# liamhebert/MultiModalDiscussionTransformer

Measured on AMD Instinct MI355X. Metric: discussion-tree comments/sec fwd+bwd, higher is better.
Workload: dtype bf16; 1 GPU; mDT-base (BERT-base + ViT-B/16 split 6+6, 6 executed graph layers, D768 H12 nb4 L100), 32 bushy 64-comment trees per GPU, 25% image comments, random-init weights, dropout 0.4/0.3/0.3 (run_train.sh:37), token lengths U{8..100} zero-padded to 100 (SURVEY.md §8d; mean 54.3 valid tokens), text side ragged: padded token positions are not computed (identical logits / gradients), last fusion layer comput; trees_per_gpu=32, parallelism=dp1, frozen_initial_encoders=False

## Files before the change

include/mdt_hip.h:

```cpp
#ifndef MDT_HIP_H
#define MDT_HIP_H

#include <stdint.h>

#ifdef __cplusplus
extern "C" {
#endif

#define MDT_ABI_VERSION 1

typedef enum { MDT_F32 = 0, MDT_BF16 = 1 } mdt_dtype;

typedef enum {
  MDT_OK = 0,
  MDT_ERR_ARG = -1,
  MDT_ERR_INVALID = MDT_ERR_ARG,
  MDT_ERR_UNSUPPORTED = -2,
  MDT_ERR_LAUNCH = -3
} mdt_status;

enum {
  MDT_EPI_BIAS = 1,
  MDT_EPI_GELU = 2,
  MDT_EPI_RESIDUAL = 4,
  MDT_EPI_DGELU = 8,
  MDT_EPI_ACCUM = 16,
  MDT_EPI_ATOMIC = 32,
  MDT_EPI_COLSUM = 128,
  MDT_EPI_AUX_GRAD = 256,
  MDT_EPI_MULAUX = 512,
  MDT_EPI_ASUM = 1024,
  MDT_EPI_DROPOUT = 64
};

int mdt_abi_version(void);
const char* mdt_last_error_string(void);
const char* mdt_last_route(void);
const char* mdt_source_hash(void);

int mdt_gemm(void* stream, int dtype, int out_dtype, int trans_a, int trans_b,
             int64_t M, int64_t N, int64_t K,
             const void* A, int64_t lda, const void* B, int64_t ldb,
             void* C, int64_t ldc, int epilogue, float alpha,
             const void* bias, const void* residual, int64_t ldr,
             void* aux, int64_t ldaux, int split_k, float drop_p, uint64_t drop_seed, float* colsum);
size_t mdt_gemm_tile_queue_bytes(void);
int mdt_gemm_set_tile_queue(void* zeroed_device_buffer, size_t bytes);
void mdt_reload_env(void);

int mdt_dropout(void* stream, int dtype, int64_t rows, int D, const void* x, int64_t ldx, void* y, int64_t ldy,
                float p, uint64_t seed);
int mdt_dropout_mask(void* stream, int64_t n, float p, uint64_t seed, uint8_t* mask);

enum { MDT_ACT_GELU = 0, MDT_ACT_RELU = 1, MDT_ACT_GELU_ACCURATE = 2, MDT_ACT_TANH = 3, MDT_ACT_LINEAR = 4 };
int mdt_act_fwd(void* stream, int dtype, int kind, int64_t rows, int N, const void* pre, int64_t ld_pre, void* h, int64_t ld_h,
                void* u, int64_t ld_u, float drop_p, uint64_t drop_seed);

int mdt_colsum(void* stream, int dtype, int64_t M, int64_t N, const void* X, int64_t ldx, float* out,
               const int32_t* row_weight);

int mdt_layernorm_fwd(void* stream, int dtype, int64_t rows, int D, const void* x, int64_t ldx,
                      const void* gamma, const void* beta, float eps,
                      void* y, int64_t ldy, float* mean, float* rstd);
int mdt_layernorm_fwd_q8(void* stream, int dtype, int64_t rows, int D, const void* x, int64_t ldx, const void* gamma,
                         const void* beta, float eps, void* y, int64_t ldy, float* mean, float* rstd, void* q8_out,
                         int64_t ld_q8, int q8_format, const float* q8_scale, float* q8_amax);
int mdt_layernorm_bwd(void* stream, int dtype, int64_t rows, int D, const void* dy, int64_t lddy,
                      const void* x, int64_t ldx, const void* gamma, const float* mean, const float* rstd,
                      const void* add, int64_t ldadd, void* dx, int64_t lddx, float* dgamma, float* dbeta,
                      void* dxd, int64_t lddxd, float drop_p, uint64_t drop_seed, float* colsum);

typedef struct {
  int dtype;
  int nseq, S, H, hd;
  int64_t seq_stride, pos_stride;
  float scale;
  const void* qkv; int64_t ld_qkv;
  void* out; int64_t ld_out;
  float* lse;
  const uint8_t* key_mask;
  const float* dense_bias;
  const float* attn_bias;
  const int32_t* spatial_pos;
  const void* sp_table;
  const void* virt;
  const uint8_t* key_pad;
  int num_spatial;
  float drop_p;
  uint64_t drop_seed;
  const int32_t* seq_offsets;
  int q_limit;
  const int32_t* seq_ids;
  int s_cap;
  int nseq_total;
} mdt_attn_fwd_args;
int mdt_attention_fwd(void* stream, const mdt_attn_fwd_args* a);

typedef struct {
  mdt_attn_fwd_args f;
  const void* dout; int64_t ld_dout;
  void* dqkv; int64_t ld_dqkv;
  float* d_dense_bias;
  float* d_sp_table;
  float* d_virt;
} mdt_attn_bwd_args;
int mdt_attention_bwd(void* stream, const mdt_attn_bwd_args* a);
int mdt_attention_route(const mdt_attn_bwd_args* a, int bwd, char* route, size_t route_bytes, int32_t geometry[2]);
int mdt_attention_mean_probs(void* stream, const mdt_attn_fwd_args* a, float* out);
int mdt_attention_head_weights(void* stream, const mdt_attn_fwd_args* a, int raw_scores, float* out);

int mdt_graph_attn_bias(void* stream, int dtype, int nseq, int S, int H, const float* attn_bias,
                        const int32_t* spatial_pos, const void* sp_table, const void* virt,
                        float* out);

int mdt_row_axpby(void* stream, int dtype, int64_t nrows, int D,
                  void* dst, int64_t ldd, const int32_t* di, int64_t d_inner, int64_t d_stride, int64_t d_off,
                  const void* a, int64_t lda, const int32_t* ai, int64_t a_inner, int64_t a_stride, int64_t a_off, float alpha,
                  const void* b, int64_t ldb, const int32_t* bi, int64_t b_inner, int64_t b_stride, int64_t b_off, float beta,
                  int accumulate);
int mdt_row_scatter_add_f32(void* stream, int dtype, int64_t nrows, int D, float* table, int64_t ldt,
                            const int32_t* idx, const void* src, int64_t lds, int64_t s_stride, int64_t s_off);

int mdt_bert_embed_sum(void* stream, int dtype, int64_t M, int L, const int32_t* ids, const int32_t* types,
                       const void* word, const void* pos, const void* type, int D,
                       void* out, int64_t ldo, int64_t out_seq_stride, int64_t out_off);

int mdt_bert_embed_rows(void* stream, int dtype, int64_t rows, const int32_t* ids, const int32_t* types,
                        const int32_t* pos_ids, const void* word, const void* pos, const void* type, int D,
                        void* out, int64_t ldo);
int mdt_bert_embed_ln_rows(void* stream, int dtype, int64_t rows, const int32_t* ids, const int32_t* types,
                           const int32_t* pos_ids, const void* word, const void* pos, const void* type, int D,
                           const void* gamma, const void* beta, float eps, void* xs, int64_t ldxs, void* y, int64_t ldy,
                           float* mean, float* rstd);

int mdt_vit_patchify(void* stream, int dtype, int I, int C, int HW, int p, const float* img, void* cols, int64_t ldc);
int mdt_vit_assemble(void* stream, int dtype, int I, int np, int D, const void* patches, int64_t ldp,
                     const void* cls, const void* pos, void* tokens, int64_t ldt, int64_t seq_stride, int64_t off);
int mdt_vit_patch_embed(void* stream, int I, int C, int HW, int p, const float* img, const void* w, int64_t ldw,
                        const void* bias, const void* cls, const void* pos, int D, void* tokens, int64_t ldt,
                        int64_t seq_stride, int64_t off);

int mdt_graph_node_feature(void* stream, int dtype, int B, int T, int D, const void* src, int64_t lds,
                           const int32_t* node_row, const int32_t* in_degree, const int32_t* out_degree,
                           const void* in_emb, const void* out_emb, const void* graph_token, void* x, int64_t ldx);

int mdt_tanh_fwd(void* stream, int dtype, int64_t n, const void* x, void* y);
int mdt_tanh_bwd(void* stream, int dtype, int64_t n, const void* y, const void* dy, void* dx);

int mdt_node_ce(void* stream, int dtype, int64_t M, int nlab, const void* logits, const int32_t* rows,
                const int32_t* targets, float w_neg, float w_pos, int fp16_loss, float grad_scale,
                float* out_loss, int32_t* counters, void* dlogits);

int mdt_gemm_fp8(void* stream, int a_format, int64_t M, int64_t N, int64_t K, const void* A, int64_t lda, const void* B,
                 int64_t ldb, void* C, int64_t ldc, int epilogue, const float* inv_scale_a, const float* inv_scale_b,
                 const void* bias, const void* residual, int64_t ldr, void* aux, int64_t ldaux, float drop_p,
                 uint64_t drop_seed, float* colsum);
int mdt_gemm_fp8_q8(void* stream, int a_format, int64_t M, int64_t N, int64_t K, const void* A, int64_t lda, const void* B,
                    int64_t ldb, void* C, int64_t ldc, int epilogue, const float* inv_scale_a, const float* inv_scale_b,
                    const void* bias, const void* residual, int64_t ldr, void* aux, int64_t ldaux, float drop_p,
                    uint64_t drop_seed, float* colsum, void* q8_out, int64_t ld_q8, int q8_format, const float* q8_scale,
                    float* q8_amax);
int mdt_fp8_quantize(void* stream, int src_dtype, int fmt, int64_t rows, int64_t cols, const void* src, int64_t ld_src,
                     void* dst, int64_t ld_dst, const float* scale_dev, float* amax_dev);
int mdt_fp8_scale_update(void* stream, int n, float* amax, float* scale, float* inv_scale, const float* fmt_max, float margin);

size_t mdt_contrastive_loss_workspace_bytes(int B, int D);
int mdt_contrastive_loss(void* stream, int dtype, int B, int D, const void* emb, int64_t ld, const float* y,
                         const float* hard_y, float scale, float soft_negative_weight, int adaptive, void* workspace,
                         float grad_scale, float* out_loss, int32_t* counters, void* d_emb, int64_t ldd);

int mdt_cast(void* stream, int src_dtype, int dst_dtype, int64_t n, const void* src, void* dst);
int mdt_transpose2d(void* stream, int src_dtype, int dst_dtype, int64_t rows, int64_t cols,
                    const void* src, int64_t lds, void* dst, int64_t ldd);

int mdt_adam_step(void* stream, int dtype, int64_t n, void* param, float* master, const float* grad, float* m,
                  float* v, float lr, float beta1, float beta2, float eps, float weight_decay, int step,
                  const float* grad_scale);

typedef struct {
  void* param;
  float* master;
  const float* grad;
  float* m;
  float* v;
  int64_t numel;
} mdt_adam_tensor;
int mdt_adam_step_multi(void* stream, int dtype, int n_tensors, const mdt_adam_tensor* table_dev,
                        const int64_t* chunk_first_dev, int64_t total_chunks, float lr, float beta1, float beta2,
                        float eps, float weight_decay, int step, const float* grad_scale);

typedef struct {
  float scale;
  float gnorm;
  float step_size;
  int32_t skip;
  int32_t applied;
  int32_t clipped;
  int32_t skipped;
  int32_t reserved;
} mdt_adam_guard;
int mdt_grad_sumsq_multi(void* stream, int n_tensors, const mdt_adam_tensor* table_dev, const int64_t* chunk_first_dev,
                         int64_t total_chunks, float* partials);
int mdt_grad_sumsq(void* stream, int64_t n, const float* grad, float* partials);
int mdt_grad_norm_finalize(void* stream, const float* partials, int64_t n_partials, float max_norm,
                           const float* grad_scale, float lr, float beta1, float beta2, int step, int reset,
                           mdt_adam_guard* guard);
int mdt_adam_step_guarded(void* stream, int dtype, int64_t n, void* param, float* master, const float* grad, float* m,
                          float* v, float lr, float beta1, float beta2, float eps, float weight_decay, int step,
                          const mdt_adam_guard* guard);
int mdt_adam_step_multi_guarded(void* stream, int dtype, int n_tensors, const mdt_adam_tensor* table_dev,
                                const int64_t* chunk_first_dev, int64_t total_chunks, float lr, float beta1, float beta2,
                                float eps, float weight_decay, int step, const mdt_adam_guard* guard);

int mdt_adam_step_ema(void* stream, int dtype, int64_t n, void* param, float* master, const float* grad, float* m,
                      float* v, float lr, float beta1, float beta2, float eps, float weight_decay, int step,
                      const float* grad_scale, float* ema, float ema_decay);
int mdt_adam_step_multi_ema(void* stream, int dtype, int n_tensors, const mdt_adam_tensor* table_dev,
                            const int64_t* chunk_first_dev, int64_t total_chunks, float lr, float beta1, float beta2,
                            float eps, float weight_decay, int step, const float* grad_scale, float* const* ema_dev,
                            float ema_decay);
int mdt_adam_step_ema_guarded(void* stream, int dtype, int64_t n, void* param, float* master, const float* grad, float* m,
                              float* v, float lr, float beta1, float beta2, float eps, float weight_decay, int step,
                              const mdt_adam_guard* guard, float* ema, float ema_decay);
int mdt_adam_step_multi_ema_guarded(void* stream, int dtype, int n_tensors, const mdt_adam_tensor* table_dev,
                                    const int64_t* chunk_first_dev, int64_t total_chunks, float lr, float beta1, float beta2,
                                    float eps, float weight_decay, int step, const mdt_adam_guard* guard, float* const* ema_dev,
                                    float ema_decay);
int mdt_ema_swap_multi(void* stream, int dtype, int n_tensors, const mdt_adam_tensor* table_dev, float* const* ema_dev,
                       const int64_t* chunk_first_dev, int64_t total_chunks, int restore);

typedef struct {
  float lr_scale;
  float weight_decay;
} mdt_adam_group;
int mdt_adam_step_multi_groups(void* stream, int dtype, int n_tensors, const mdt_adam_tensor* table_dev,
                               const int64_t* chunk_first_dev, int64_t total_chunks, float lr, float beta1, float beta2,
                               float eps, int step, const mdt_adam_group* groups_dev, const float* grad_scale,
                               const mdt_adam_guard* guard, float* const* ema_dev, float ema_decay);
int mdt_adam_step_group(void* stream, int dtype, int64_t n, void* param, float* master, const float* grad, float* m, float* v,
                        float lr, float beta1, float beta2, float eps, int step, float lr_scale, float weight_decay,
                        const float* grad_scale, const mdt_adam_guard* guard, float* ema, float ema_decay);

int mdt_sum_slices_f32(void* stream, int64_t rows, int64_t cols, int slices, const float* ws, int64_t ld_ws, int64_t slice_stride,
                       float* out, int64_t ldo, int accumulate);
size_t mdt_gemm_splitk_ordered_workspace_bytes(int64_t M, int64_t N, int split_k);
int mdt_gemm_splitk_ordered(void* stream, int dtype, int trans_a, int trans_b, int64_t M, int64_t N, int64_t K,
                            const void* A, int64_t lda, const void* B, int64_t ldb, float* C, int64_t ldc, float alpha,
                            int split_k, void* workspace, size_t workspace_bytes);
size_t mdt_colsum_ordered_workspace_bytes(int64_t M, int64_t N);
int mdt_colsum_ordered(void* stream, int dtype, int64_t M, int64_t N, const void* X, int64_t ldx, float* out,
                       const int32_t* row_weight, void* workspace, size_t workspace_bytes);
size_t mdt_layernorm_bwd_ordered_workspace_bytes(int64_t rows, int D);
int mdt_layernorm_bwd_ordered(void* stream, int dtype, int64_t rows, int D, const void* dy, int64_t lddy,
                              const void* x, int64_t ldx, const void* gamma, const float* mean, const float* rstd,
                              const void* add, int64_t ldadd, void* dx, int64_t lddx, float* dgamma, float* dbeta,
                              void* dxd, int64_t lddxd, float drop_p, uint64_t drop_seed, float* colsum,
                              void* workspace, size_t workspace_bytes);
int mdt_row_segment_sum_f32(void* stream, int dtype, int nseg, int D, float* table, int64_t ldt, const int32_t* seg_row,
                            const int32_t* seg_off, const int32_t* order, const void* src, int64_t lds, int64_t s_stride,
                            int64_t s_off);
// ... 40 lines not shown
```

multimodaldiscussiontransformer_amd/_lib.py:

```python
from __future__ import annotations

import ctypes as C
import os
import sys

import torch

_HERE = os.path.dirname(os.path.abspath(__file__))
LIB_PATH = os.path.join(_HERE, "libmdt_hip.so")

MDT_F32, MDT_BF16 = 0, 1
EPI_BIAS, EPI_GELU, EPI_RESIDUAL, EPI_DGELU, EPI_ACCUM, EPI_ATOMIC, EPI_DROPOUT, EPI_COLSUM = 1, 2, 4, 8, 16, 32, 64, 128
EPI_AUX_GRAD, EPI_MULAUX, EPI_ASUM = 256, 512, 1024
ACT_GELU, ACT_RELU, ACT_GELU_ACCURATE, ACT_TANH, ACT_LINEAR = 0, 1, 2, 3, 4

_vp, _i, _i64, _f = C.c_void_p, C.c_int, C.c_int64, C.c_float


class AttnFwdArgs(C.Structure):
    _fields_ = [
        ("dtype", _i), ("nseq", _i), ("S", _i), ("H", _i), ("hd", _i),
        ("seq_stride", _i64), ("pos_stride", _i64), ("scale", _f),
        ("qkv", _vp), ("ld_qkv", _i64), ("out", _vp), ("ld_out", _i64), ("lse", _vp),
        ("key_mask", _vp), ("dense_bias", _vp), ("attn_bias", _vp), ("spatial_pos", _vp),
        ("sp_table", _vp), ("virt", _vp), ("key_pad", _vp), ("num_spatial", _i),
        ("drop_p", _f), ("drop_seed", C.c_uint64), ("seq_offsets", _vp), ("q_limit", _i),
        ("seq_ids", _vp), ("s_cap", _i), ("nseq_total", _i),
    ]


class AttnBwdArgs(C.Structure):
    _fields_ = [
        ("f", AttnFwdArgs), ("dout", _vp), ("ld_dout", _i64), ("dqkv", _vp), ("ld_dqkv", _i64),
        ("d_dense_bias", _vp), ("d_sp_table", _vp), ("d_virt", _vp),
    ]


_SIGS = {
    "mdt_abi_version": ([], _i),
    "mdt_last_error_string": ([], C.c_char_p),
    "mdt_last_route": ([], C.c_char_p),
    "mdt_source_hash": ([], C.c_char_p),
    "mdt_gemm": ([_vp, _i, _i, _i, _i, _i64, _i64, _i64, _vp, _i64, _vp, _i64, _vp, _i64, _i, _f, _vp, _vp, _i64,
                  _vp, _i64, _i, _f, C.c_uint64, _vp], _i),
    "mdt_gemm_tile_queue_bytes": ([], C.c_size_t),
    "mdt_gemm_set_tile_queue": ([_vp, C.c_size_t], _i),
    "mdt_reload_env": ([], None),
    "mdt_dropout": ([_vp, _i, _i64, _i, _vp, _i64, _vp, _i64, _f, C.c_uint64], _i),
    "mdt_dropout_mask": ([_vp, _i64, _f, C.c_uint64, _vp], _i),
    "mdt_act_fwd": ([_vp, _i, _i, _i64, _i, _vp, _i64, _vp, _i64, _vp, _i64, _f, C.c_uint64], _i),
    "mdt_colsum": ([_vp, _i, _i64, _i64, _vp, _i64, _vp, _vp], _i),
    "mdt_layernorm_fwd": ([_vp, _i, _i64, _i, _vp, _i64, _vp, _vp, _f, _vp, _i64, _vp, _vp], _i),
    "mdt_layernorm_fwd_q8": ([_vp, _i, _i64, _i, _vp, _i64, _vp, _vp, _f, _vp, _i64, _vp, _vp, _vp, _i64, _i, _vp, _vp], _i),
    "mdt_layernorm_bwd": ([_vp, _i, _i64, _i, _vp, _i64, _vp, _i64, _vp, _vp, _vp, _vp, _i64, _vp, _i64, _vp, _vp,
                           _vp, _i64, _f, C.c_uint64, _vp], _i),
    "mdt_attention_fwd": ([_vp, C.POINTER(AttnFwdArgs)], _i),
    "mdt_attention_bwd": ([_vp, C.POINTER(AttnBwdArgs)], _i),
    "mdt_attention_route": ([C.POINTER(AttnBwdArgs), _i, C.c_char_p, C.c_size_t, C.POINTER(C.c_int32)], _i),
    "mdt_attention_mean_probs": ([_vp, C.POINTER(AttnFwdArgs), _vp], _i),
    "mdt_attention_head_weights": ([_vp, C.POINTER(AttnFwdArgs), _i, _vp], _i),
    "mdt_graph_attn_bias": ([_vp, _i, _i, _i, _i, _vp, _vp, _vp, _vp, _vp], _i),
    "mdt_row_axpby": ([_vp, _i, _i64, _i, _vp, _i64, _vp, _i64, _i64, _i64, _vp, _i64, _vp, _i64, _i64, _i64, _f,
                       _vp, _i64, _vp, _i64, _i64, _i64, _f, _i], _i),
    "mdt_row_scatter_add_f32": ([_vp, _i, _i64, _i, _vp, _i64, _vp, _vp, _i64, _i64, _i64], _i),
    "mdt_sum_slices_f32": ([_vp, _i64, _i64, _i, _vp, _i64, _i64, _vp, _i64, _i], _i),
    "mdt_gemm_splitk_ordered_workspace_bytes": ([_i64, _i64, _i], C.c_size_t),
    "mdt_gemm_splitk_ordered": ([_vp, _i, _i, _i, _i64, _i64, _i64, _vp, _i64, _vp, _i64, _vp, _i64, _f, _i, _vp, C.c_size_t], _i),
    "mdt_colsum_ordered_workspace_bytes": ([_i64, _i64], C.c_size_t),
    "mdt_colsum_ordered": ([_vp, _i, _i64, _i64, _vp, _i64, _vp, _vp, _vp, C.c_size_t], _i),
    "mdt_layernorm_bwd_ordered_workspace_bytes": ([_i64, _i], C.c_size_t),
    "mdt_layernorm_bwd_ordered": ([_vp, _i, _i64, _i, _vp, _i64, _vp, _i64, _vp, _vp, _vp, _vp, _i64, _vp, _i64, _vp, _vp,
                                   _vp, _i64, _f, C.c_uint64, _vp, _vp, C.c_size_t], _i),
    "mdt_row_segment_sum_f32": ([_vp, _i, _i, _i, _vp, _i64, _vp, _vp, _vp, _vp, _i64, _i64, _i64], _i),
    "mdt_attn_bias_grad_ordered_workspace_bytes": ([_i, _i, _i], C.c_size_t),
    "mdt_attn_bias_grad_ordered": ([_vp, _i, _i, _i, _i, _vp, _vp, _vp, _vp, _vp, C.c_size_t], _i),
    "mdt_float_atomic_launches": ([_i], _i64),
    "mdt_lora_down": ([_vp, _i, _i64, _i, _i, _vp, _i64, _vp, _i64, _vp, _i64, _f], _i),
    "mdt_lora_up_add": ([_vp, _i, _i64, _i, _i, _vp, _i64, _vp, _i64, _vp, _i64, _f], _i),
    "mdt_lora_up_add_drop": ([_vp, _i, _i64, _i, _i, _vp, _i64, _vp, _i64, _vp, _i64, _f, _f, C.c_uint64], _i),
    "mdt_lora_up_add_mul": ([_vp, _i, _i64, _i, _i, _vp, _i64, _vp, _i64, _vp, _i64, _vp, _i64, _f], _i),
    "mdt_lora_up_act": ([_vp, _i, _i, _i64, _i, _i, _vp, _i64, _vp, _i64, _vp, _i64, _vp, _i64, _vp, _i64, _f, _f, C.c_uint64], _i),
    "mdt_lora_wgrad_slab_rows": ([], _i),
    "mdt_lora_wgrad_workspace_bytes": ([_i64, _i, _i], C.c_size_t),
    "mdt_lora_wgrad": ([_vp, _i, _i64, _i, _i, _vp, _i64, _vp, _i64, _vp, _i64, _f, _vp, C.c_size_t], _i),
    "mdt_bert_embed_sum": ([_vp, _i, _i64, _i, _vp, _vp, _vp, _vp, _vp, _i, _vp, _i64, _i64, _i64], _i),
    "mdt_bert_embed_rows": ([_vp, _i, _i64, _vp, _vp, _vp, _vp, _vp, _vp, _i, _vp, _i64], _i),
    "mdt_bert_embed_ln_rows": ([_vp, _i, _i64, _vp, _vp, _vp, _vp, _vp, _vp, _i, _vp, _vp, _f, _vp, _i64, _vp, _i64, _vp, _vp], _i),
    "mdt_vit_patchify": ([_vp, _i, _i, _i, _i, _i, _vp, _vp, _i64], _i),
    "mdt_vit_assemble": ([_vp, _i, _i, _i, _i, _vp, _i64, _vp, _vp, _vp, _i64, _i64, _i64], _i),
    "mdt_vit_patch_embed": ([_vp, _i, _i, _i, _i, _vp, _vp, _i64, _vp, _vp, _vp, _i, _vp, _i64, _i64, _i64], _i),
    "mdt_graph_node_feature": ([_vp, _i, _i, _i, _i, _vp, _i64, _vp, _vp, _vp, _vp, _vp, _vp, _vp, _i64], _i),
    "mdt_tanh_fwd": ([_vp, _i, _i64, _vp, _vp], _i),
    "mdt_tanh_bwd": ([_vp, _i, _i64, _vp, _vp, _vp], _i),
    "mdt_node_ce": ([_vp, _i, _i64, _i, _vp, _vp, _vp, _f, _f, _i, _f, _vp, _vp, _vp], _i),
    "mdt_gemm_fp8": ([_vp, _i, _i64, _i64, _i64, _vp, _i64, _vp, _i64, _vp, _i64, _i, _vp, _vp, _vp, _vp, _i64, _vp, _i64, _f,
                      C.c_uint64, _vp], _i),
    "mdt_gemm_fp8_q8": ([_vp, _i, _i64, _i64, _i64, _vp, _i64, _vp, _i64, _vp, _i64, _i, _vp, _vp, _vp, _vp, _i64, _vp, _i64, _f,
                         C.c_uint64, _vp, _vp, _i64, _i, _vp, _vp], _i),
    "mdt_fp8_quantize": ([_vp, _i, _i, _i64, _i64, _vp, _i64, _vp, _i64, _vp, _vp], _i),
    "mdt_fp8_scale_update": ([_vp, _i, _vp, _vp, _vp, _vp, _f], _i),
    "mdt_contrastive_loss_workspace_bytes": ([_i, _i], C.c_size_t),
    "mdt_contrastive_loss": ([_vp, _i, _i, _i, _vp, _i64, _vp, _vp, _f, _f, _i, _vp, _f, _vp, _vp, _vp, _i64], _i),
    "mdt_adam_step_multi": ([_vp, _i, _i, _vp, _vp, _i64, _f, _f, _f, _f, _f, _i, _vp], _i),
    "mdt_cast": ([_vp, _i, _i, _i64, _vp, _vp], _i),
    "mdt_transpose2d": ([_vp, _i, _i, _i64, _i64, _vp, _i64, _vp, _i64], _i),
    "mdt_adam_step": ([_vp, _i, _i64, _vp, _vp, _vp, _vp, _vp, _f, _f, _f, _f, _f, _i, _vp], _i),
    "mdt_grad_sumsq_multi": ([_vp, _i, _vp, _vp, _i64, _vp], _i),
    "mdt_grad_sumsq": ([_vp, _i64, _vp, _vp], _i),
    "mdt_grad_norm_finalize": ([_vp, _vp, _i64, _f, _vp, _f, _f, _f, _i, _i, _vp], _i),
    "mdt_adam_step_guarded": ([_vp, _i, _i64, _vp, _vp, _vp, _vp, _vp, _f, _f, _f, _f, _f, _i, _vp], _i),
    "mdt_adam_step_multi_guarded": ([_vp, _i, _i, _vp, _vp, _i64, _f, _f, _f, _f, _f, _i, _vp], _i),
    "mdt_adam_step_ema": ([_vp, _i, _i64, _vp, _vp, _vp, _vp, _vp, _f, _f, _f, _f, _f, _i, _vp, _vp, _f], _i),
    "mdt_adam_step_multi_ema": ([_vp, _i, _i, _vp, _vp, _i64, _f, _f, _f, _f, _f, _i, _vp, _vp, _f], _i),
    "mdt_adam_step_ema_guarded": ([_vp, _i, _i64, _vp, _vp, _vp, _vp, _vp, _f, _f, _f, _f, _f, _i, _vp, _vp, _f], _i),
    "mdt_adam_step_multi_ema_guarded": ([_vp, _i, _i, _vp, _vp, _i64, _f, _f, _f, _f, _f, _i, _vp, _vp, _f], _i),
    "mdt_adam_step_multi_groups": ([_vp, _i, _i, _vp, _vp, _i64, _f, _f, _f, _f, _i, _vp, _vp, _vp, _vp, _f], _i),
    "mdt_adam_step_group": ([_vp, _i, _i64, _vp, _vp, _vp, _vp, _vp, _f, _f, _f, _f, _i, _f, _f, _vp, _vp, _vp, _f], _i),
    "mdt_ema_swap_multi": ([_vp, _i, _i, _vp, _vp, _vp, _i64, _i], _i),
    "mdt_resize_plan_ksize": ([_i, _i], _i),
    "mdt_resize_plan": ([_i, _i, _vp, _vp, _i], _i),
    "mdt_image_norm_lut": ([C.c_double, _vp, _vp, _vp], _i),
    "mdt_image_preprocess": ([_vp, _i, _i, _vp, _vp, _vp, _vp, _vp, _i, _vp, _vp, _i], _i),
    "mdt_pack_structure": ([_i, _vp, _vp, _i, _i, _vp, _vp, _vp], _i),
    "mdt_pack_structure_ud": ([_i, _vp, _vp, _vp, _i, _i, _vp, _vp, _vp], _i),
}

EXPORTS = tuple(_SIGS)


class MdtError(RuntimeError):
    status = 0


class MdtUnsupported(MdtError):
    status = -2


def _load():
    if not os.path.exists(LIB_PATH):
        raise ImportError(
            f"{LIB_PATH} is missing: the HIP extension is the product path and has no fallback. "
            "Build it with `python -m multimodaldiscussiontransformer_amd.build` (hipcc, gfx950).")
    lib = C.CDLL(LIB_PATH)
    for name, (args, res) in _SIGS.items():
        fn = getattr(lib, name)
        fn.argtypes = args
        fn.restype = res
    if lib.mdt_abi_version() != 1:
        raise ImportError("libmdt_hip.so ABI version mismatch")
    skip = os.environ.get("MDT_SKIP_SOURCE_HASH") == "1"
    if skip and ("pytest" in sys.modules or os.environ.get("MDT_BENCH_OFFICIAL") == "1"):
        raise ImportError("MDT_SKIP_SOURCE_HASH=1 is refused under pytest and bench.py (bench.py --foreign-library for an A/B arm)")
    from .build import source_hash, hash_inputs_present
    if not skip and hash_inputs_present():
        built, here = lib.mdt_source_hash().decode(), source_hash()
        if built != here:
            raise ImportError(f"{LIB_PATH} was built from other sources (library {built[:16]}, csrc/ {here[:16]}): rebuild with "
                              "`python -m multimodaldiscussiontransformer_amd.build` (MDT_SKIP_SOURCE_HASH=1 overrides, for A/B runs of two builds)")
    return lib


lib = _load()


def reload_env():
    lib.mdt_reload_env()


def last_route() -> str:
    return lib.mdt_last_route().decode()


_TILE_QUEUE = None


def enable_dynamic_tile_queue(device="cuda"):
    global _TILE_QUEUE
    if _TILE_QUEUE is None:
        _TILE_QUEUE = torch.zeros(lib.mdt_gemm_tile_queue_bytes() // 4, dtype=torch.int32, device=device)
        check(lib.mdt_gemm_set_tile_queue(_TILE_QUEUE.data_ptr(), _TILE_QUEUE.numel() * 4), "mdt_gemm_set_tile_queue")
    return _TILE_QUEUE


def check(status: int, what: str = ""):
    if status != 0:
        e = (MdtUnsupported if status == -2 else MdtError)(f"{what}: status {status}: {lib.mdt_last_error_string().decode()}")
        e.status = status
        raise e


def dt(t: torch.Tensor) -> int:
    if t.dtype == torch.float32:
        return MDT_F32
    if t.dtype == torch.bfloat16:
        return MDT_BF16
    raise MdtError(f"unsupported dtype {t.dtype} (fp32 and bf16 only)")


def ptr(t) -> int:
    if t is None:
        return None
    if not t.is_cuda:
        raise MdtError("libmdt_hip operates on device tensors only (no CPU path)")
    return t.data_ptr()


def stream() -> int:
    if not torch.cuda.is_available():
        raise MdtError("no GPU visible: libmdt_hip is the only compute path (there is no CPU fallback)")
    return torch.cuda.current_stream().cuda_stream
```

multimodaldiscussiontransformer_amd/build.py:

```python
from __future__ import annotations

import os
import subprocess
import sys
from concurrent.futures import ThreadPoolExecutor

HERE = os.path.dirname(os.path.abspath(__file__))
CSRC = os.path.join(HERE, "csrc")
OUT = os.path.join(HERE, "libmdt_hip.so")
SOURCES = ["gemm.hip", "gemm_wgrad.hip", "gemm_f8.hip", "layernorm.hip", "attention.hip", "attention_v2.hip", "attention_long.hip", "rowops.hip", "elementwise.hip", "ordered.hip", "lora.hip", "activation.hip", "patch_embed.hip", "contrastive.hip", "fp8.hip", "optim.hip", "image.hip", "host.cpp"]
FLAGS = ["--offload-arch=gfx950", "-O3", "-fPIC", "-std=c++17", "-Wno-unused-result", "-ffp-contract=off"]
EXTRA = {"attention.hip": ["-mllvm", "-amdgpu-mfma-vgpr-form=1"], "attention_v2.hip": ["-mllvm", "-amdgpu-mfma-vgpr-form=1"],
         "gemm_wgrad.hip": ["-mllvm", "-amdgpu-mfma-vgpr-form=1"]}


def source_hash() -> str:
    import hashlib
    h = hashlib.sha256()
    files = sorted(os.path.join(CSRC, f) for f in os.listdir(CSRC) if f.endswith((".hip", ".cpp", ".hpp", ".h")))
    files.append(os.path.join(HERE, "..", "include", "mdt_hip.h"))
    for f in files:
        h.update(os.path.basename(f).encode() + b"\0")
        h.update(open(f, "rb").read())
    return h.hexdigest()


def hash_inputs_present() -> bool:
    return os.path.isdir(CSRC) and os.path.exists(os.path.join(HERE, "..", "include", "mdt_hip.h"))


def _stale(target, deps):
    if not os.path.exists(target):
        return True
    t = os.path.getmtime(target)
    return any(os.path.getmtime(d) > t for d in deps)


def build(verbose: bool = False, force: bool = False) -> str:
    hipcc = os.environ.get("HIPCC", "/opt/rocm/bin/hipcc")
    objdir = os.path.join(HERE, "build")
    os.makedirs(objdir, exist_ok=True)
    headers = [os.path.join(CSRC, "common.hpp"), os.path.join(CSRC, "attention_common.hpp"), os.path.join(CSRC, "gemm_tiles.hpp"), os.path.join(CSRC, "gemm_epilogue.hpp"),
               os.path.join(HERE, "..", "include", "mdt_hip.h")]
    objs, jobs = [], []
    for s in SOURCES:
        src = os.path.join(CSRC, s)
        obj = os.path.join(objdir, s.rsplit(".", 1)[0] + ".o")
        objs.append(obj)
        if force or _stale(obj, [src] + headers):
            lang = ["-x", "hip"] if s.endswith(".cpp") else []
            jobs.append([hipcc] + FLAGS + EXTRA.get(s, []) + lang + ["-c", src, "-o", obj])

    def run(cmd):
        if verbose:
            print(" ".join(cmd), flush=True)
        r = subprocess.run(cmd, capture_output=True, text=True)
        if r.returncode != 0:
            raise RuntimeError("hipcc failed:\n" + " ".join(cmd) + "\n" + r.stdout + r.stderr)
        return r

    with ThreadPoolExecutor(max_workers=4) as ex:
        list(ex.map(run, jobs))
    digest = source_hash()
    stamp_src = os.path.join(objdir, "source_hash.cpp")
    stamp_obj = os.path.join(objdir, "source_hash.o")
    text = f'extern "C" const char* mdt_source_hash(void) {{ return "{digest}"; }}\n'
    if not os.path.exists(stamp_src) or open(stamp_src).read() != text or not os.path.exists(stamp_obj):
        open(stamp_src, "w").write(text)
        run([hipcc, "-x", "c++", "-O1", "-fPIC", "-c", stamp_src, "-o", stamp_obj])
        jobs.append(None)
    if force or jobs or _stale(OUT, objs + [stamp_obj]):
        run([hipcc, "--offload-arch=gfx950", "-shared", "-fPIC", "-o", OUT] + objs + [stamp_obj])
    return OUT


if __name__ == "__main__":
    print(build(verbose=True, force="--force" in sys.argv))
```

multimodaldiscussiontransformer_amd/csrc/attention.hip:

```cpp
#include <type_traits>

#include <stdlib.h>

#include "attention_common.hpp"

namespace mdt {

template <typename T> struct MM;
template <> struct MM<float> {
  static constexpr int KS = 4;
  typedef float frag;
  static __device__ __forceinline__ f32x4 mma(frag a, frag b, f32x4 c) { return mfma_f32(a, b, c); }
};
template <> struct MM<bf16_t> {
  static constexpr int KS = 32;
  typedef bf16x8 frag;
  static __device__ __forceinline__ f32x4 mma(frag a, frag b, f32x4 c) { return mfma_bf16(a, b, c); }
};

template <typename T> struct Src {
  const T* p;
  int64_t ld;
  int rows;
};
// ... 471 lines not shown
  AttnPlan pl{};
  pl.bwd = bwd;
  pl.st_bias = a.attn_bias != nullptr;
  pl.drop = a.drop_p > 0.f;
  pl.binned = a.seq_ids != nullptr || a.s_cap > 0;
  pl.dense_only = (a.dense_bias != nullptr || p.d_dense_bias != nullptr) && !pl.st_bias;
  pl.cap = a.s_cap > 0 ? a.s_cap : a.S;
  pl.n_t = (pl.cap + 15) / 16;
  pl.nhist = (bwd && pl.st_bias) ? attn_hist_size(a.num_spatial) : 0;
  const bool bf = a.dtype == MDT_BF16;
  if (pl.binned) {
    if (a.S > 272 || !bf || a.hd != 64 || !a.seq_offsets) {
      set_error("attention: seq_ids / s_cap are for ragged bf16 launches with head_dim 64 and S <= 272");
      return refuse(pl);
    }
  } else if (a.S > 272) return plan_long(pl, a);
  if (!attn_head_dim_ok(a.hd)) {
    set_error(bf ? "attention(bf16): head_dim %d unsupported (16, 64, 96 or 128)" : "attention: head_dim %d unsupported (16, 64, 96 or 128)", a.hd);
    return refuse(pl);
  }
  if (bf && pl.dense_only && !attn_v1_fits(a.hd, a.S)) return plan_long(pl, a);
  const bool one_pass = a.hd == 64 && !pl.st_bias && !pl.dense_only && attn_one_pass_lds_bytes(pl.n_t) <= ATTN_LDS_MAX && pl.n_t <= 16;
  pl.rows_img = attn_one_pass_rows(pl.n_t);
  pl.ldq = attn_one_pass_ldq(pl.n_t);
  auto ok = [&](AttnRoute r) {
    switch (r) {
      case AttnRoute::v1: return !pl.binned && a.q_limit == 0 && attn_v1_fits(a.hd, a.S);
      case AttnRoute::v2: return !pl.binned && !pl.dense_only && a.q_limit == 0 && a.S <= 112;
      case AttnRoute::v3: return !pl.dense_only;
      case AttnRoute::v4: return one_pass;
      case AttnRoute::v4x: return one_pass && pl.n_t <= 2 * V4_EXACT_PAIRS;
      case AttnRoute::v5: return one_pass && pl.n_t > 8 && pl.rows_img * 8 <= 4 * 512;
      default: return false;
    }
  };
  if (!bf) pl.route = AttnRoute::v1;
  else if (!bwd) pl.route = pl.dense_only ? AttnRoute::v1 : AttnRoute::v2;
  else {
    const AttnRoute family = ok(AttnRoute::v5) ? AttnRoute::v5 : ok(AttnRoute::v4x) ? AttnRoute::v4x : one_pass ? AttnRoute::v4 : AttnRoute::v3;
    if (pl.binned) pl.route = family;
    else if (pl.dense_only) pl.route = AttnRoute::v1;
    else if (a.S > 256) pl.route = family;
    else if (a.S <= 80 && a.q_limit == 0 && pl.st_bias) pl.route = AttnRoute::v1;
    else if (!pl.drop && ok(AttnRoute::v2)) pl.route = AttnRoute::v2;
    else pl.route = family;
    const AttnRoute forced = switches().attn_bwd;
    if (forced != AttnRoute::none && ok(forced)) pl.route = forced;
  }
  switch (pl.route) {
    case AttnRoute::v1: {
      pl.rung = attn_rung<2, 5, 7, 9, 13, 17>((a.S + 15) / 16);
      if (!pl.rung) { set_error("attention: S=%d exceeds the 272-token limit of the single-pass kernel", a.S); return refuse(pl); }
      const size_t lds = attn_v1_lds_bytes(bf, a.hd, pl.rung, bwd, pl.nhist);
      if (lds > ATTN_LDS_MAX) {
        set_error(bwd ? "attention_bwd (v1): S=%d with head_dim %d needs %zu bytes of LDS" : "attention (v1): S=%d with head_dim %d needs %zu bytes of LDS", a.S, a.hd, lds);
        return refuse(pl);
      }
      if (!bf && bwd && a.hd > 64 && pl.rung == 17 && pl.st_bias && pl.drop) return plan_long(pl, a);
      break;
    }
    case AttnRoute::v2:
      pl.rung = attn_rung<2, 4, 5, 7, 9, 13, 17>(pl.n_t);
      if (!pl.rung) { set_error("attention_v2: S=%d exceeds 272", a.S); return refuse(pl); }
      if (bwd && pl.rung > 7) { set_error("attention_v2: backward supports S <= 112 (got %d)", a.S); return refuse(pl); }
      if (!bwd) pl.waves = attn_v2_fwd_waves(pl.rung, pl.st_bias);
      break;
    case AttnRoute::v3: {
      pl.tight = attn_v3_tight(a.hd, pl.cap);
      pl.s_pad = attn_v3_s_pad(pl.cap, pl.tight);
      const size_t lds = attn_v3_lds_bytes(a.hd, pl.s_pad, pl.tight, pl.nhist);
      if (lds > ATTN_LDS_MAX) { set_error("attention_bwd_v3: S=%d needs %zu bytes of LDS", pl.cap, lds); return refuse(pl); }
      pl.threads = (a.hd <= 64 && !pl.st_bias && pl.s_pad > 128) ? 512 : 256;
      break;
    }
    case AttnRoute::v5:
      pl.items = (int)((int64_t)a.H * a.nseq);
      pl.wgs = pl.items < device_cus() ? pl.items : device_cus();
      break;
    case AttnRoute::v4:
    case AttnRoute::v4x:
      pl.waves = pl.n_t <= 4 ? 4 : pl.n_t <= 8 ? 8 : 16;
      break;
    default: break;
  }
  return pl;
}

int attention_v1_launch(hipStream_t st, const AttnParams& p, const AttnPlan& pl) {
  return with_dtype(p.f.dtype, [&](auto t) { return with_head_dim(p.f.hd, [&](auto hd) { return with_flags(pl, [&](auto s, auto d) {
    return with_rung<2, 5, 7, 9, 13, 17>(pl.rung, [&](auto nt) {
      using T = typename decltype(t)::type;
      constexpr int HD = decltype(hd)::value, NT = decltype(nt)::value;
      constexpr bool STRUCT = decltype(s)::value, DROP = decltype(d)::value, BF = !std::is_same<T, float>::value;
      const size_t lds = attn_v1_lds_bytes(BF, HD, NT, pl.bwd, pl.nhist);
      const dim3 grid(p.f.H, p.f.nseq);
      if (!pl.bwd) return launch_route<attn_fwd_kernel<T, HD, NT, STRUCT, DROP>>("v1", grid, 256, lds, st, p);
      if constexpr (!BF && HD > 64 && NT == 17 && STRUCT && DROP) return attn_unplanned("the fp32 v1 backward of wide heads at 17 tiles with structural bias and dropout");
      else return launch_route<attn_bwd_kernel<T, HD, NT, STRUCT, DROP>>("v1", grid, 256, lds, st, p);
    });
  }); }); });
}

static bool attn_rows_aligned(int dtype, const void* base, int64_t ld) {
  return dtype == MDT_BF16 ? (ld % 8 == 0 && ((uintptr_t)base & 15) == 0) : ((uintptr_t)base & 3) == 0;
}

static int check_args(const mdt_attn_fwd_args& a) {
  MDT_CHECK_ARG(a.dtype == MDT_F32 || a.dtype == MDT_BF16, "attention: bad dtype %d", a.dtype);
  MDT_CHECK_ARG(a.nseq >= 0 && a.S > 0 && a.H > 0 && a.hd > 0, "attention: bad shape nseq=%d S=%d H=%d hd=%d", a.nseq,
                a.S, a.H, a.hd);
  MDT_CHECK_ARG(a.qkv && a.out && a.lse, "attention: null qkv / out / lse");
  MDT_CHECK_ARG(a.ld_qkv >= 3 * a.H * a.hd && a.ld_out >= a.H * a.hd, "attention: row strides too small");
  if (a.dtype == MDT_BF16) {
    MDT_CHECK_ARG(attn_rows_aligned(a.dtype, a.qkv, a.ld_qkv), "attention(bf16): qkv must be 16-byte aligned rows");
    MDT_CHECK_ARG(attn_rows_aligned(a.dtype, a.out, a.ld_out), "attention(bf16): out must be 16-byte aligned rows");
  } else {
    MDT_CHECK_ARG(attn_rows_aligned(a.dtype, a.qkv, a.ld_qkv), "attention(fp32): qkv must be 4-byte aligned");
    MDT_CHECK_ARG(attn_rows_aligned(a.dtype, a.out, a.ld_out), "attention(fp32): out must be 4-byte aligned");
  }
  if (a.attn_bias) MDT_CHECK_ARG(a.spatial_pos && a.sp_table && a.virt && a.num_spatial > 0, "attention: incomplete structural bias");
  MDT_CHECK_ARG(a.drop_p >= 0.f && a.drop_p < 1.f, "attention: dropout p=%f out of [0,1)", a.drop_p);
  if (a.seq_offsets)
    MDT_CHECK_ARG(a.pos_stride == 1 && !a.key_mask && !a.key_pad && !a.dense_bias && !a.attn_bias,
                  "attention: ragged sequences (seq_offsets) take no masks / biases and need pos_stride == 1");
  MDT_CHECK_ARG(a.s_cap >= 0 && a.s_cap <= a.S, "attention: s_cap=%d outside [0, S=%d]", a.s_cap, a.S);
  MDT_CHECK_ARG(!a.seq_ids || (a.seq_offsets && (a.nseq_total == 0 || a.nseq_total >= a.nseq)),
                "attention: seq_ids need seq_offsets (and nseq_total >= nseq)");
  MDT_CHECK_ARG(a.drop_p == 0.f || (uint64_t)(a.nseq_total > a.nseq ? a.nseq_total : a.nseq) * a.H * a.S * (a.S + 1) < (1ull << 32),
                "attention: dropout counters are 32-bit (nseq*H*S*(S+1) must stay below 2^32)");
  return MDT_OK;
}

static int checked_params(const mdt_attn_fwd_args& f, const mdt_attn_bwd_args* b, AttnParams& p) {
  if (int e = check_args(f)) return e;
  memset(&p, 0, sizeof(p));
  p.f = f;
  p.drop = make_drop(f.drop_p, f.drop_seed);
  if (!b) return MDT_OK;
  MDT_CHECK_ARG(b->dout && b->dqkv, "attention_bwd: null dout / dqkv");
  MDT_CHECK_ARG(b->ld_dqkv >= 3 * f.H * f.hd, "attention_bwd: ld_dqkv too small");
  MDT_CHECK_ARG(b->ld_dout >= f.H * f.hd, "attention_bwd: ld_dout too small");
  if (f.dtype == MDT_BF16) {
    MDT_CHECK_ARG(attn_rows_aligned(f.dtype, b->dout, b->ld_dout), "attention_bwd(bf16): dout must be 16-byte aligned rows");
    MDT_CHECK_ARG(attn_rows_aligned(f.dtype, b->dqkv, b->ld_dqkv), "attention_bwd(bf16): dqkv must be 16-byte aligned rows");
  } else {
    MDT_CHECK_ARG(attn_rows_aligned(f.dtype, b->dout, b->ld_dout), "attention_bwd(fp32): dout must be 4-byte aligned");
    MDT_CHECK_ARG(attn_rows_aligned(f.dtype, b->dqkv, b->ld_dqkv), "attention_bwd(fp32): dqkv must be 4-byte aligned");
  }
  p.dout = b->dout; p.ld_dout = b->ld_dout; p.dqkv = b->dqkv; p.ld_dqkv = b->ld_dqkv;
  p.d_dense_bias = b->d_dense_bias; p.d_sp_table = b->d_sp_table; p.d_virt = b->d_virt;
  return MDT_OK;
}

static int dispatch(hipStream_t st, const mdt_attn_fwd_args& f, const mdt_attn_bwd_args* b) {
  AttnParams p;
  if (int e = checked_params(f, b, p)) return e;
  if (p.d_sp_table || p.d_virt) note_float_atomic_launch();
  const AttnPlan pl = attn_plan(p, b != nullptr);
  if (pl.status != MDT_OK) return pl.status;
  switch (pl.route) {
    case AttnRoute::v1: return attention_v1_launch(st, p, pl);
    case AttnRoute::long_: return attention_long_launch(st, p, pl);
    default: return attention_v2_launch(st, p, pl);
  }
}

}

using namespace mdt;

extern "C" int mdt_attention_fwd(void* stream, const mdt_attn_fwd_args* a) {
  MDT_CHECK_ARG(a, "attention_fwd: null args");
  if (a->nseq == 0) return MDT_OK;
  return dispatch((hipStream_t)stream, *a, nullptr);
}

extern "C" int mdt_attention_bwd(void* stream, const mdt_attn_bwd_args* a) {
  MDT_CHECK_ARG(a, "attention_bwd: null args");
  if (a->f.nseq == 0) return MDT_OK;
  return dispatch((hipStream_t)stream, a->f, a);
}

extern "C" int mdt_attention_route(const mdt_attn_bwd_args* a, int bwd, char* route, size_t route_bytes, int32_t geometry[2]) {
  MDT_CHECK_ARG(a && route && route_bytes > 0 && geometry, "attention_route: null args");
  route[0] = 0;
  geometry[0] = geometry[1] = 0;
  AttnParams p;
  if (int e = checked_params(a->f, bwd ? a : nullptr, p)) return e;
  const AttnPlan pl = attn_plan(p, bwd != 0);
  if (pl.status != MDT_OK) return pl.status;
  snprintf(route, route_bytes, "%s", route_name(pl.route));
  switch (pl.route) {
    case AttnRoute::v1:
    case AttnRoute::v2: geometry[0] = pl.rung; geometry[1] = pl.waves; break;
    case AttnRoute::v3: geometry[0] = pl.s_pad; geometry[1] = pl.threads; break;
    case AttnRoute::v4:
    case AttnRoute::v4x: geometry[0] = pl.waves; break;
    default: break;
  }
  return MDT_OK;
}

extern "C" int mdt_attention_mean_probs(void* stream, const mdt_attn_fwd_args* a, float* out) {
  MDT_CHECK_ARG(a && out, "attention_mean_probs: null args");
  if (a->nseq == 0) return MDT_OK;
  if (int e = check_args(*a)) return e;
  MDT_CHECK_ARG(!a->seq_offsets, "attention_mean_probs: ragged sequences are not supported (module-level API only)");
  const int64_t n = (int64_t)a->nseq * a->S * a->S;
  const int grid = (int)((n + 255) / 256 > 8192 ? 8192 : (n + 255) / 256);
  return with_dtype(a->dtype, [&](auto t) {
    return launch_plain<attn_mean_probs_kernel<typename decltype(t)::type>>("attention_mean_probs", grid, 256, (hipStream_t)stream, *a, out);
  });
}

template <typename T, bool RAW>
__global__ __launch_bounds__(256) void attn_head_weights_kernel(mdt_attn_fwd_args a, float* out) {
  const int S = a.S, H = a.H, hd = a.hd;
  const int64_t n = (int64_t)a.nseq * H * S * S;
  for (int64_t i = (int64_t)blockIdx.x * 256 + threadIdx.x; i < n; i += (int64_t)gridDim.x * 256) {
    const int key = (int)(i % S), q = (int)((i / S) % S), h = (int)((i / ((int64_t)S * S)) % H), seq = (int)(i / ((int64_t)S * S * H));
    const T* qrow = (const T*)a.qkv + ((int64_t)seq * a.seq_stride + (int64_t)q * a.pos_stride) * a.ld_qkv + h * hd;
    const T* krow = (const T*)a.qkv + ((int64_t)seq * a.seq_stride + (int64_t)key * a.pos_stride) * a.ld_qkv + (int64_t)H * hd + h * hd;
    const BiasCtx bc = bias_ctx(a, seq, h, S);
    float v = key_only_bias<T>(bc, key);
    if (v == 0.f) {
      float dot = 0.f;
      for (int d = 0; d < hd; ++d) dot += to_f32(qrow[d]) * to_f32(krow[d]);
      v = dot * a.scale + (a.attn_bias ? pair_bias<T, true>(bc, q, key) : pair_bias<T, false>(bc, q, key));
    }
    if constexpr (RAW) {
      out[i] = v;
    } else {
      const float l = a.lse[((int64_t)seq * H + h) * S + q];
      out[i] = (v == -INFINITY || l == -INFINITY) ? 0.f : __expf(v - l);
    }
  }
}

extern "C" int mdt_attention_head_weights(void* stream, const mdt_attn_fwd_args* a, int raw_scores, float* out) {
  MDT_CHECK_ARG(a && out, "attention_head_weights: null args");
  if (a->nseq == 0) return MDT_OK;
  if (int e = check_args(*a)) return e;
  MDT_CHECK_ARG(!a->seq_offsets, "attention_head_weights: ragged sequences are not supported (module-level API only)");
  MDT_CHECK_ARG(raw_scores || a->lse, "attention_head_weights: probabilities need the forward's log-sum-exp");
  const int64_t n = (int64_t)a->nseq * a->H * a->S * a->S;
  const int grid = (int)((n + 255) / 256 > 8192 ? 8192 : (n + 255) / 256);
  hipStream_t st = (hipStream_t)stream;
  return with_dtype(a->dtype, [&](auto t) {
    using T = typename decltype(t)::type;
    return raw_scores ? launch_plain<attn_head_weights_kernel<T, true>>("attention_head_weights", grid, 256, st, *a, out)
                      : launch_plain<attn_head_weights_kernel<T, false>>("attention_head_weights", grid, 256, st, *a, out);
  });
}

extern "C" int mdt_graph_attn_bias(void* stream, int dtype, int nseq, int S, int H, const float* attn_bias,
                                   const int32_t* spatial_pos, const void* sp_table, const void* virt, float* out) {
  MDT_CHECK_ARG(attn_bias && spatial_pos && sp_table && virt && out, "graph_attn_bias: null pointer");
  if (nseq == 0) return MDT_OK;
  const int64_t n = (int64_t)nseq * H * S * S;
  const int grid = (int)((n + 255) / 256 > 8192 ? 8192 : (n + 255) / 256);
  hipStream_t st = (hipStream_t)stream;
  return with_dtype(dtype, [&](auto t) {
    using T = typename decltype(t)::type;
    return launch_plain<graph_attn_bias_kernel<T>>("graph_attn_bias", grid, 256, st, nseq, S, H, attn_bias, spatial_pos, (const T*)sp_table, (const T*)virt, out);
  });
}
```

multimodaldiscussiontransformer_amd/csrc/attention_common.hpp:

```cpp
#pragma once
#include "common.hpp"

namespace mdt {

struct AttnParams {
  mdt_attn_fwd_args f;
  DropCfg drop;
  const void* dout; int64_t ld_dout;
  void* dqkv; int64_t ld_dqkv;
  float* d_dense_bias; float* d_sp_table; float* d_virt;
};

struct BiasCtx {
  int seq, h, S, H;
  const uint8_t* key_mask;
  const uint8_t* key_pad;
  const float* dense;
  const float* attn_bias;
  const int32_t* sp;
  const void* table;
  const void* virt;
};
__device__ __forceinline__ BiasCtx bias_ctx(const mdt_attn_fwd_args& a, int seq, int h, int S) {
  return BiasCtx{seq, h, S, a.H, a.key_mask, a.key_pad, a.dense_bias, a.attn_bias, a.spatial_pos, a.sp_table, a.virt};
}

template <typename T>
struct AttnItem {
  int seq, S, SL, D;
  int64_t row0;
  const T* qkv; const T* dout; const T* out; T* dqkv;
  int64_t tld, dld, old_, gld;
};
template <typename T, int HD>
__device__ __forceinline__ AttnItem<T> attn_item(const AttnParams& P, int h, unsigned si) {
  const mdt_attn_fwd_args& a = P.f;
  const int seq = a.seq_ids ? a.seq_ids[si] : (int)si;
  const int SL = a.S, D = a.H * HD;
  const int S = a.seq_offsets ? a.seq_offsets[seq + 1] - a.seq_offsets[seq] : a.S;
  const int64_t row0 = a.seq_offsets ? (int64_t)a.seq_offsets[seq] : (int64_t)seq * a.seq_stride;
  const T* qkv = (const T*)a.qkv + row0 * a.ld_qkv + h * HD;
  const T* dout = (const T*)P.dout + row0 * P.ld_dout + h * HD;
  const T* out = (const T*)a.out + row0 * a.ld_out + h * HD;
  T* dqkv = (T*)P.dqkv + row0 * P.ld_dqkv + h * HD;
  return AttnItem<T>{seq, S, SL, D, row0, qkv, dout, out, dqkv, a.pos_stride * a.ld_qkv, a.pos_stride * P.ld_dout, a.pos_stride * a.ld_out,
                     a.pos_stride * P.ld_dqkv};
}

template <typename T>
__device__ __forceinline__ float key_only_bias(const BiasCtx& b, int key) {
  if (key >= b.S) return -INFINITY;
  if (b.key_mask && !b.key_mask[(int64_t)b.seq * b.S + key]) return -INFINITY;
  if (b.key_pad && b.key_pad[(int64_t)b.seq * b.S + key]) return -INFINITY;
  return 0.f;
}

template <typename T, bool STRUCT>
__device__ __forceinline__ float pair_bias(const BiasCtx& b, int q, int key) {
  float v = 0.f;
  if (b.dense) v += b.dense[(((int64_t)b.seq * b.H + b.h) * b.S + q) * b.S + key];
  if constexpr (STRUCT) {
    v += 2.0f * b.attn_bias[((int64_t)b.seq * b.S + q) * b.S + key];
    if (q >= 1 && key >= 1) {
      const int idx = b.sp[((int64_t)b.seq * (b.S - 1) + (q - 1)) * (b.S - 1) + (key - 1)];
      v += to_f32(((const T*)b.table)[(int64_t)idx * b.H + b.h]);
    } else {
      v += to_f32(((const T*)b.virt)[b.h]);
    }
  }
  return v;
}

constexpr float LOG2E = 1.4426950408889634f, LN2 = 0.6931471805599453f;

__device__ __forceinline__ uint32_t attn_row_pairs(int bh, int S, int q) {
  return (uint32_t)(bh * S + q) * (uint32_t)((S + 1) >> 1);
}
__device__ __forceinline__ uint32_t attn_drop_word(const DropCfg& d, uint32_t row_pairs, int key) {
  return drop_mix((row_pairs + (uint32_t)(key >> 1)) ^ d.key);
}
__device__ __forceinline__ bool drop_keep_lo(const DropCfg& d, uint32_t w) { return (w & 0xFFFFu) >= d.thresh; }
__device__ __forceinline__ bool drop_keep_hi(const DropCfg& d, uint32_t w) { return (w >> 16) >= d.thresh; }
__device__ __forceinline__ void attn_keep4_keys(const DropCfg& d, uint32_t pair, bool (&keep)[4]) {
  const uint32_t w0 = drop_mix(pair ^ d.key), w1 = drop_mix((pair + 1) ^ d.key);
  keep[0] = drop_keep_lo(d, w0); keep[1] = drop_keep_hi(d, w0);
  keep[2] = drop_keep_lo(d, w1); keep[3] = drop_keep_hi(d, w1);
}
__device__ __forceinline__ void attn_keep4_queries(const DropCfg& d, uint32_t kh, int qb, uint32_t s2h, int odd, bool (&keep)[4]) {
  const uint32_t ra = kh + (uint32_t)(qb + 2 * odd) * s2h;
  const uint32_t wa = drop_mix(ra ^ d.key), wb = drop_mix((ra + s2h) ^ d.key);
  const uint32_t pa = (uint32_t)__builtin_amdgcn_update_dpp(0, (int)wa, 0xB1, 0xF, 0xF, false);
  const uint32_t pb = (uint32_t)__builtin_amdgcn_update_dpp(0, (int)wb, 0xB1, 0xF, 0xF, false);
  const uint32_t w[4] = {odd ? pa : wa, odd ? pb : wb, odd ? wa : pa, odd ? wb : pb};
#pragma unroll
  for (int r = 0; r < 4; ++r) keep[r] = ((w[r] >> (16 * odd)) & 0xFFFFu) >= d.thresh;
}
__device__ __forceinline__ float attn_drop_scale(const DropCfg& d, int bh, int S, int q, int key) {
  const uint32_t w = attn_drop_word(d, attn_row_pairs(bh, S, q), key);
  return ((key & 1) ? drop_keep_hi(d, w) : drop_keep_lo(d, w)) ? d.inv_keep : 0.f;
}

__host__ __device__ inline int attn_hist_size(int num_spatial) { return (num_spatial + 1 + 3) & ~3; }
template <bool STRUCT>
__device__ __forceinline__ void attn_bias_grad_add(const AttnParams& P, float* s_hist, int seq, int h, int S, int q, int key, float ds) {
  const mdt_attn_fwd_args& a = P.f;
  if (P.d_dense_bias) P.d_dense_bias[(((int64_t)seq * a.H + h) * S + q) * S + key] = ds;
  if constexpr (STRUCT) {
    if (P.d_sp_table && ds != 0.f) {
      if (q >= 1 && key >= 1) {
        const int idx = a.spatial_pos[((int64_t)seq * (S - 1) + (q - 1)) * (S - 1) + (key - 1)];
        if (idx != 0) atomicAdd(s_hist + idx, ds);
      } else {
        atomicAdd(s_hist + a.num_spatial, ds);
      }
    }
  }
}
__device__ __forceinline__ void attn_bias_grad_flush(const AttnParams& P, const float* s_hist, int h, int tid, int nthr) {
  const mdt_attn_fwd_args& a = P.f;
  if (P.d_sp_table) {
    for (int i = tid; i <= a.num_spatial; i += nthr) {
      const float v = s_hist[i];
      if (v != 0.f) {
        if (i < a.num_spatial) atomicAdd(P.d_sp_table + (int64_t)i * a.H + h, v);
        else if (P.d_virt) atomicAdd(P.d_virt + h, v);
      }
    }
  }
}

constexpr int attn_v1_ld(int hd) { return hd >= 32 ? hd + 8 : hd; }
constexpr int attn_v2_ld(int hd, bool tight) { return hd < 32 ? hd : (hd <= 64 || tight) ? hd + 8 : hd + 16; }
template <int HD, bool TIGHT = false> constexpr int v2_ld = attn_v2_ld(HD, TIGHT);
template <int HD, int NT> constexpr int v2_ld_nt = v2_ld<HD, (HD == 128 && NT > 16)>;
constexpr int V4_EXACT_PAIRS = 3;
constexpr size_t ATTN_LDS_MAX = 160 * 1024;

constexpr bool attn_v1_fits(int hd, int S) { return hd < 128 || S <= 208; }

constexpr size_t attn_v1_lds_bytes(bool bf, int hd, int nt, bool bwd, int nhist) {
  const int s_pad32 = (nt * 16 + 31) & ~31, sld = s_pad32 + (bf ? 8 : 1);
  return (bwd ? (size_t)(2 * s_pad32 + nhist) * 4 : 0) + (size_t)4 * 16 * sld * (bf ? 2 : 4) + (bf ? (size_t)2 * s_pad32 * attn_v1_ld(hd) * 2 : 0);
}
constexpr size_t attn_v2_lds_bytes(int hd, int nt, bool bwd, int nhist) {
  const int s_pad = ((nt + 1) / 2) * 32;
  return (size_t)2 * s_pad * attn_v2_ld(hd, !bwd && hd == 128 && nt > 16) * 2 + (size_t)(bwd ? 3 : 1) * s_pad * 4 + (size_t)nhist * 4 + (bwd ? 0 : 16);
}
constexpr bool attn_v3_tight(int hd, int cap) { return hd == 128 && cap > 256; }
constexpr int attn_v3_s_pad(int cap, bool tight) { return tight ? (cap + 31) & ~31 : (cap + 63) & ~63; }
constexpr size_t attn_v3_lds_bytes(int hd, int s_pad, bool tight, int nhist) {
  return (size_t)2 * s_pad * attn_v2_ld(hd, tight) * 2 + (size_t)3 * s_pad * 4 + (size_t)nhist * 4;
}
constexpr int attn_one_pass_rows(int n_t) { return ((n_t + 1) / 2) * 32; }
constexpr int attn_one_pass_ldq(int n_t) { return (n_t & 1) ? 16 * n_t : 16 * n_t + 16; }
constexpr size_t attn_one_pass_lds_bytes(int n_t) {
  const size_t rows = attn_one_pass_rows(n_t), slabs = n_t <= 2 * V4_EXACT_PAIRS ? 7 : 0;
  return 2 * rows * attn_v2_ld(64, false) * 2 + (3 + slabs) * rows * 4 + (size_t)16 * n_t * attn_one_pass_ldq(n_t) * 2;
}
constexpr int attn_v2_fwd_waves(int nt, bool st_bias) { return (nt >= 13 && !st_bias) ? 8 : 4; }

struct AttnPlan {
  int status;
  AttnRoute route;
  bool bwd, st_bias, drop, binned, dense_only;
  int cap, n_t;
  int nhist;
  int rung;
  int s_pad, threads; bool tight;
  int rows_img, ldq, waves;
  int items, wgs;
};
AttnPlan attn_plan(const AttnParams& p, bool bwd);
int attention_v1_launch(hipStream_t st, const AttnParams& p, const AttnPlan& pl);
int attention_v2_launch(hipStream_t st, const AttnParams& p, const AttnPlan& pl);
int attention_long_launch(hipStream_t st, const AttnParams& p, const AttnPlan& pl);
inline int attn_unplanned(const char* what) { set_error("attention: %s is not instantiated and attn_plan never plans it", what); return MDT_ERR_UNSUPPORTED; }

constexpr bool attn_head_dim_ok(int hd) { return hd == 16 || hd == 64 || hd == 96 || hd == 128; }
template <typename F>
static int with_head_dim(int hd, F&& f) {
  switch (hd) {
    case 16: return f(std::integral_constant<int, 16>{});
    case 64: return f(std::integral_constant<int, 64>{});
    case 96: return f(std::integral_constant<int, 96>{});
    case 128: return f(std::integral_constant<int, 128>{});
  }
  return attn_unplanned("this head width");
}
template <typename F>
static int with_flags(const AttnPlan& pl, F&& f) {
  using T = std::true_type;
  using N = std::false_type;
  if (pl.st_bias && pl.drop) return f(T{}, T{});
  if (pl.st_bias) return f(T{}, N{});
  if (pl.drop) return f(N{}, T{});
  return f(N{}, N{});
}
template <int... RUNGS>
constexpr int attn_rung(int nt) {
  int r = 0;
  ((r = (r == 0 && nt <= RUNGS) ? RUNGS : r), ...);
  return r;
}
template <int... RUNGS, typename F>
static int with_rung(int rung, F&& f) {
  int e = MDT_ERR_UNSUPPORTED;
  const bool hit = ((rung == RUNGS ? (e = f(std::integral_constant<int, RUNGS>{}), true) : false) || ...);
  return hit ? e : attn_unplanned("this key-tile rung");
}

}
```

multimodaldiscussiontransformer_amd/csrc/attention_v2.hip:

```cpp
#include <type_traits>

#include "attention_common.hpp"

namespace mdt {

template <int HD> constexpr int v2_ks = (HD + 31) / 32;

template <int HD, int LD = v2_ld<HD>>
__device__ __forceinline__ void v2_stage(bf16_t* img, const bf16_t* g, int64_t g_ld, int S, int rows_pad, int tid, int nthr = 256) {
  constexpr int CH = HD / 8;
  for (int e = tid; e < rows_pad * CH; e += nthr) {
    const int r = e / CH, c = e - r * CH;
    bf16x8 v = bf16x8{0, 0, 0, 0, 0, 0, 0, 0};
    if (r < S) v = *(const bf16x8*)(g + r * g_ld + c * 8);
    *(bf16x8*)(img + r * LD + c * 8) = v;
  }
}

template <int HD, int NCH>
__device__ __forceinline__ void v2_stage_req(bf16x8 (&v)[NCH], const bf16_t* g, int64_t g_ld, int S, int tid, int nthr) {
  constexpr int CH = HD / 8;
#pragma unroll
  for (int j = 0; j < NCH; ++j) {
    const int e = tid + j * nthr, r = e / CH, c = e - r * CH;
    v[j] = *(const bf16x8*)(g + (r < S ? r : S - 1) * g_ld + c * 8);
  }
}
template <int HD, int NCH, int LD = v2_ld<HD>>
__device__ __forceinline__ void v2_stage_put(bf16_t* img, const bf16x8 (&v)[NCH], int S, int rows_pad, int tid, int nthr, bf16_t* spare) {
  constexpr int CH = HD / 8;
#pragma unroll
  for (int j = 0; j < NCH; ++j) {
    const int e = tid + j * nthr, r = e / CH, c = e - r * CH;
    bf16_t* dst = e < rows_pad * CH ? img + r * LD + c * 8 : spare;
    *(bf16x8*)dst = r < S ? v[j] : bf16x8{0, 0, 0, 0, 0, 0, 0, 0};
  }
}
struct KeyBytes { uint8_t km, kp; };
__device__ __forceinline__ KeyBytes key_only_bias_req(const BiasCtx& b, int key, const void* readable) {
  KeyBytes k{1, 0};
  if (b.key_mask || b.key_pad) {
    const int64_t at = (int64_t)b.seq * b.S + (key < b.S ? key : b.S - 1);
    const uint8_t* pm = b.key_mask ? b.key_mask + at : (const uint8_t*)readable;
    const uint8_t* pp = b.key_pad ? b.key_pad + at : (const uint8_t*)readable;
    const uint8_t m = *pm, q = *pp;
    k = KeyBytes{(uint8_t)(b.key_mask ? m : 1), (uint8_t)(b.key_pad ? q : 0)};
  }
  return k;
}
__device__ __forceinline__ float key_only_bias_of(const BiasCtx& b, int key, KeyBytes k) {
  return (key < b.S && k.km && !k.kp) ? 0.f : -INFINITY;
}

template <int HD>
__device__ __forceinline__ int v2_chunk(int lane) {
  static_assert(HD % 32 == 0 || HD == 16, "a head is whole K = 32 steps, or half of one");
  return HD % 32 == 0 ? lane >> 4 : (lane >> 4) & (HD / 8 - 1);
}
template <int HD, int LD = v2_ld<HD>>
__device__ __forceinline__ bf16x8 v2_frag_lds(const bf16_t* img, int rc0, int k0, int lane) {
  const bf16_t* a = img + (rc0 + (lane & 15)) * LD + k0 + 8 * v2_chunk<HD>(lane);
  return *(const __attribute__((address_space(3))) bf16x8*)LDS_PTR(a);
}
template <int HD>
__device__ __forceinline__ bf16x8 v2_frag_glb(const bf16_t* p, int64_t ld, int rows, int rc0, int k0, int lane) {
  int rc = rc0 + (lane & 15);
  if (rc > rows - 1) rc = rows - 1;
  bf16x8 v = *(const bf16x8*)(p + rc * ld + k0 + 8 * v2_chunk<HD>(lane));
  if constexpr (HD % 32 != 0) {
    if (k0 + 8 * (lane >> 4) >= HD) v = bf16x8{0, 0, 0, 0, 0, 0, 0, 0};
  }
  return v;
}
template <int HD, int LD = v2_ld<HD>>
__device__ __forceinline__ bf16x8 v2_frag_tr(const bf16_t* img, int t0, int d0, int lane) {
  const int g = lane >> 4, q4 = (lane >> 2) & 3, pp = lane & 3;
  const bf16_t* a = img + (t0 * 16 + 4 * g + q4) * LD + d0 + pp * 4;
  const bf16x4 lo = lds_read_tr16(a);
  const bf16x4 hi = lds_read_tr16(a + 16 * LD);
  return bf16x8{lo[0], lo[1], lo[2], lo[3], hi[0], hi[1], hi[2], hi[3]};
}
__device__ __forceinline__ bf16x8 v2_pack(const f32x4& lo, const f32x4& hi) {
  return bf16x8{(bf16_t)lo[0], (bf16_t)lo[1], (bf16_t)lo[2], (bf16_t)lo[3],
                (bf16_t)hi[0], (bf16_t)hi[1], (bf16_t)hi[2], (bf16_t)hi[3]};
}
__device__ __forceinline__ float col_max(float v) {
  v = fmaxf(v, __shfl_xor(v, 16, 64));
  return fmaxf(v, __shfl_xor(v, 32, 64));
}
__device__ __forceinline__ float col_sum(float v) {
  v += __shfl_xor(v, 16, 64);
  return v + __shfl_xor(v, 32, 64);
}

struct Row32 { bf16x8 a, b; };
__device__ __forceinline__ int rows4_off(int g) { return 16 * (g & 1) + 8 * (g >> 1); }
__device__ __forceinline__ Row32 rows4_exchange(const f32x4 (&x)[4], float scale) {
  uint32_t lo[4], hi[4];
#pragma unroll
  for (int d = 0; d < 4; ++d) {
    const bf16x4 v = bf16x4{(bf16_t)(x[d][0] * scale), (bf16_t)(x[d][1] * scale), (bf16_t)(x[d][2] * scale), (bf16_t)(x[d][3] * scale)};
    const uint2 u = __builtin_bit_cast(uint2, v);
    lo[d] = u.x;
    hi[d] = u.y;
  }
  asm volatile("s_nop 1\n\tv_permlane16_swap_b32 %0, %1" : "+v"(lo[0]), "+v"(lo[1]));
  asm volatile("s_nop 1\n\tv_permlane16_swap_b32 %0, %1" : "+v"(hi[0]), "+v"(hi[1]));
  asm volatile("s_nop 1\n\tv_permlane16_swap_b32 %0, %1" : "+v"(lo[2]), "+v"(lo[3]));
  asm volatile("s_nop 1\n\tv_permlane16_swap_b32 %0, %1" : "+v"(hi[2]), "+v"(hi[3]));
  Row32 r;
  r.a = __builtin_bit_cast(bf16x8, uint4{lo[0], hi[0], lo[1], hi[1]});
  r.b = __builtin_bit_cast(bf16x8, uint4{lo[2], hi[2], lo[3], hi[3]});
  return r;
}
__device__ __forceinline__ void rows4_store(bf16_t* row, const Row32& v, int g) {
  *(bf16x8*)(row + rows4_off(g)) = v.a;
  *(bf16x8*)(row + rows4_off(g) + 32) = v.b;
}
__device__ __forceinline__ void row_piece(bf16_t* p, const f32x4& x, float scale) {
  *(bf16x4*)p = bf16x4{(bf16_t)(x[0] * scale), (bf16_t)(x[1] * scale), (bf16_t)(x[2] * scale), (bf16_t)(x[3] * scale)};
}

template <bool STRUCT>
__device__ __forceinline__ void v2_p_ds(f32x4& sc, f32x4& dp, float scale2, float kb, const f32x4& l2v, const f32x4& dlv, const bool (&keep)[4],
                                        const BiasCtx* bc = nullptr, int qb = 0, int key = 0, bool kok = false) {
#pragma unroll
  for (int r = 0; r < 4; ++r) {
    float v = __builtin_fmaf(sc[r], scale2, kb);
    if constexpr (STRUCT) {
      const int q = qb + r;
      if (kok && q < bc->S) v = __builtin_fmaf(pair_bias<bf16_t, true>(*bc, q, key), LOG2E, v);
    }
    const float p = __builtin_amdgcn_exp2f(v - l2v[r]);
    const float dpv = keep[r] ? dp[r] : 0.f;
    sc[r] = keep[r] ? p : 0.f;
    dp[r] = p * (dpv - dlv[r]);
  }
}

template <int HD, int NT, bool STRUCT, bool DROP, int NW>
__global__ __launch_bounds__(NW * 64) void attn_fwd_v2_kernel(AttnParams P) {
  constexpr int ND = HD / 16, NP = (NT + 1) / 2, S_PAD = NP * 32, LD = v2_ld_nt<HD, NT>;
  extern __shared__ __attribute__((aligned(16))) char smem[];
  const mdt_attn_fwd_args& a = P.f;
  const int tid = threadIdx.x, lane = tid & 63, wave = tid >> 6;
  const int h = blockIdx.x, seq = a.seq_ids ? a.seq_ids[blockIdx.y] : (int)blockIdx.y;
  const int SL = a.S, D = a.H * HD;
  const int S = a.seq_offsets ? a.seq_offsets[seq + 1] - a.seq_offsets[seq] : a.S;
  const int64_t row0 = a.seq_offsets ? (int64_t)a.seq_offsets[seq] : (int64_t)seq * a.seq_stride;
  if (S > NT * 16 || S <= 0) return;
  const bf16_t* qkv = (const bf16_t*)a.qkv + row0 * a.ld_qkv + h * HD;
  const int64_t tld = a.pos_stride * a.ld_qkv;
  bf16_t* imgK = (bf16_t*)smem;
  bf16_t* imgV = imgK + S_PAD * LD;
  float* s_kb = (float*)(imgV + S_PAD * LD);
  BiasCtx bc{seq, h, S, a.H, a.key_mask, a.key_pad, a.dense_bias, a.attn_bias, a.spatial_pos, a.sp_table, a.virt};
  const int ntk = (S + 15) >> 4;
  constexpr int MAXT = (NT + NW - 1) / NW;
  int n_qt = (S + 15) >> 4;
  if (a.q_limit > 0 && ((a.q_limit + 15) >> 4) < n_qt) n_qt = (a.q_limit + 15) >> 4;
  constexpr bool PFQ = !(HD > 64 && STRUCT && NT >= 13);
  bf16x8 fq_all[PFQ ? MAXT : 1][v2_ks<HD>];
#pragma unroll
  for (int k = 0; k < (PFQ ? MAXT : 0); ++k) {
    const int qt_k = wave + NW * k;
    if (qt_k < n_qt) {
#pragma unroll
      for (int ks = 0; ks < v2_ks<HD>; ++ks) fq_all[k][ks] = v2_frag_glb<HD>(qkv, tld, S, qt_k * 16, ks * 32, lane);
    }
  }
  {
    constexpr int NCH = (S_PAD * (HD / 8) + NW * 64 - 1) / (NW * 64), NKB = (S_PAD + NW * 64 - 1) / (NW * 64);
    bf16x8 ck[NCH], cv[NCH];
    KeyBytes kbv[NKB];
    v2_stage_req<HD, NCH>(ck, qkv + D, tld, S, tid, NW * 64);
    v2_stage_req<HD, NCH>(cv, qkv + 2 * D, tld, S, tid, NW * 64);
#pragma unroll
    for (int j = 0; j < NKB; ++j) kbv[j] = key_only_bias_req(bc, tid + j * NW * 64, qkv);
    v2_stage_put<HD, NCH, LD>(imgK, ck, S, S_PAD, tid, NW * 64, (bf16_t*)(s_kb + S_PAD));
    v2_stage_put<HD, NCH, LD>(imgV, cv, S, S_PAD, tid, NW * 64, (bf16_t*)(s_kb + S_PAD));
#pragma unroll
    for (int j = 0; j < NKB; ++j)
      if (tid + j * NW * 64 < S_PAD) s_kb[tid + j * NW * 64] = key_only_bias_of(bc, tid + j * NW * 64, kbv[j]);
  }
  __syncthreads();
  const int drop_bh = seq * a.H + h;
  const float scale2 = a.scale * LOG2E;
  const int g = lane >> 4, c = lane & 15;
#pragma unroll
  for (int k = 0; k < MAXT; ++k) {
    const int qt = wave + NW * k;
    if (qt >= n_qt) break;
    const int q0 = qt * 16;
    const int q = q0 + c;
    const int qc = q < S ? q : S - 1;
    bf16x8 fq[v2_ks<HD>];
#pragma unroll
    for (int ks = 0; ks < v2_ks<HD>; ++ks) {
      if constexpr (PFQ) fq[ks] = fq_all[k][ks];
      else fq[ks] = v2_frag_glb<HD>(qkv, tld, S, q0, ks * 32, lane);
    }
    f32x4 sc[2 * NP];
#pragma unroll
    for (int t = 0; t < 2 * NP; ++t) sc[t] = f32x4{0.f, 0.f, 0.f, 0.f};
#pragma unroll
    for (int t = 0; t < NT; ++t) {
#pragma unroll
      for (int ks = 0; ks < v2_ks<HD>; ++ks) {
        sc[t] = mfma_bf16(v2_frag_lds<HD, LD>(imgK, t * 16, ks * 32, lane), fq[ks], sc[t]);
        if (ks == v2_ks<HD> - 1 && (t & 1)) __builtin_amdgcn_sched_barrier(0);
      }
    }
    float mx = -INFINITY;
#pragma unroll
    for (int t = 0; t < NT; ++t) {
      if (t >= ntk) continue;
      const f32x4 kb = *(const f32x4*)(s_kb + t * 16 + 4 * g);
#pragma unroll
      for (int r = 0; r < 4; ++r) {
        float v = __builtin_fmaf(sc[t][r], scale2, kb[r]);
        if constexpr (STRUCT) {
          const int key = t * 16 + 4 * g + r;
          if (key < S) v = __builtin_fmaf(pair_bias<bf16_t, true>(bc, qc, key), LOG2E, v);
        }
        sc[t][r] = v;
        mx = fmaxf(mx, v);
      }
    }
    mx = col_max(mx);
    const float mxc = (mx == -INFINITY) ? 0.f : mx;
    float sum = 0.f;
#pragma unroll
    for (int t = 0; t < NT; ++t) {
      if (t >= ntk) continue;
#pragma unroll
      for (int r = 0; r < 4; ++r) {
        const float e = __builtin_amdgcn_exp2f(sc[t][r] - mxc);
        sc[t][r] = e;
        sum += e;
      }
    }
    sum = col_sum(sum);
    if (g == 0 && q < S) a.lse[((int64_t)seq * a.H + h) * SL + q] = (sum > 0.f) ? (mxc + __builtin_amdgcn_logf(sum)) * LN2 : -INFINITY;
    float inv = (sum > 0.f) ? __builtin_amdgcn_rcpf(sum) : 0.f;
    if constexpr (DROP) {
      inv *= P.drop.inv_keep;
      const uint32_t rp = attn_row_pairs(drop_bh, SL, qc) + 2 * g;
#pragma unroll
      for (int t = 0; t < NT; ++t) {
        if (t >= ntk) continue;
        const uint32_t w0 = drop_mix((rp + 8 * t) ^ P.drop.key), w1 = drop_mix((rp + 8 * t + 1) ^ P.drop.key);
        sc[t][0] = drop_keep_lo(P.drop, w0) ? sc[t][0] : 0.f;
        sc[t][1] = drop_keep_hi(P.drop, w0) ? sc[t][1] : 0.f;
        sc[t][2] = drop_keep_lo(P.drop, w1) ? sc[t][2] : 0.f;
        sc[t][3] = drop_keep_hi(P.drop, w1) ? sc[t][3] : 0.f;
      }
    }
    f32x4 o[ND];
#pragma unroll
    for (int d = 0; d < ND; ++d) o[d] = f32x4{0.f, 0.f, 0.f, 0.f};
#pragma unroll
    for (int pi = 0; pi < NP; ++pi) {
      if (2 * pi >= ntk) continue;
      const bf16x8 fp = v2_pack(sc[2 * pi], sc[2 * pi + 1]);
#pragma unroll
      for (int d = 0; d < ND; ++d) o[d] = mfma_bf16(v2_frag_tr<HD, LD>(imgV, 2 * pi, d * 16, lane), fp, o[d]);
      __builtin_amdgcn_sched_barrier(0);
    }
    if constexpr (ND == 4) {
      const Row32 ov = rows4_exchange(o, inv);
      if (q < S) {
        bf16_t* orow = (bf16_t*)a.out + (row0 + (int64_t)q * a.pos_stride) * a.ld_out + h * HD + rows4_off(g);
        *(bf16x8*)orow = ov.a;
// ... 561 lines not shown
  const float scale2 = a.scale * LOG2E;
  const int n_tq = (a.q_limit > 0 && ((a.q_limit + 15) >> 4) < n_t) ? (a.q_limit + 15) >> 4 : n_t;
  const int n_pair_q = (n_tq + 1) >> 1, n_pair_k = (n_t + 1) >> 1;

  const int odd = c & 1;
  const uint32_t base_rp = (uint32_t)(drop_bh * SL) * s2h;
  if (kt < n_t) {
    const int key = key0 + c;
    const bool kok = key < S;
    const float kb = s_kb[key];
    const uint32_t kh = base_rp + (uint32_t)(key >> 1);
    bf16_t* ds_row = dsT + (key0 + c) * ldq + 4 * g;
    f32x4 dv[ND], dk[ND];
#pragma unroll
    for (int d = 0; d < ND; ++d) { dv[d] = f32x4{0.f, 0.f, 0.f, 0.f}; dk[d] = f32x4{0.f, 0.f, 0.f, 0.f}; }
    if constexpr (EXACT) {
      f32x4 pA[V4_EXACT_PAIRS][2], dA[V4_EXACT_PAIRS][2];
      unsigned keepA[V4_EXACT_PAIRS];
#pragma unroll
      for (int pr = 0; pr < V4_EXACT_PAIRS; ++pr) {
        keepA[pr] = 0xFFu;
#pragma unroll
        for (int t = 0; t < 2; ++t) { pA[pr][t] = f32x4{0.f, 0.f, 0.f, 0.f}; dA[pr][t] = f32x4{0.f, 0.f, 0.f, 0.f}; }
        if (pr < n_pair_q) {
          const int t0 = 2 * pr;
#pragma unroll
          for (int t = 0; t < 2; ++t)
#pragma unroll
            for (int ks = 0; ks < v2_ks<HD>; ++ks) {
              pA[pr][t] = mfma_bf16(v2_frag_lds<HD>(img0, (t0 + t) * 16, ks * 32, lane), fk[ks], pA[pr][t]);
              dA[pr][t] = mfma_bf16(v2_frag_lds<HD>(img1, (t0 + t) * 16, ks * 32, lane), fv[ks], dA[pr][t]);
            }
#pragma unroll
          for (int t = 0; t < 2; ++t) {
            const int qb = (t0 + t) * 16 + 4 * g;
            const f32x4 l2v = *(const f32x4*)(s_lse + qb);
            bool keep[4] = {true, true, true, true};
            if constexpr (DROP) {
              attn_keep4_queries(P.drop, kh, qb, s2h, odd, keep);
#pragma unroll
              for (int r = 0; r < 4; ++r)
                if (!keep[r]) keepA[pr] &= ~(1u << (4 * t + r));
            }
            float x[4];
#pragma unroll
            for (int r = 0; r < 4; ++r) {
              const float v = __builtin_fmaf(pA[pr][t][r], scale2, kb);
              const float p = __builtin_amdgcn_exp2f(v - l2v[r]);
              const float dpv = keep[r] ? dA[pr][t][r] : 0.f;
              pA[pr][t][r] = p;
              dA[pr][t][r] = dpv;
              x[r] = row16_sum_dpp(p * dpv);
            }
            if (c == 0) *(f32x4*)(s_delta + kt * rows_img + qb) = f32x4{x[0], x[1], x[2], x[3]};
          }
        }
      }
      __syncthreads();
#pragma unroll
      for (int pr = 0; pr < V4_EXACT_PAIRS; ++pr) {
        if (pr < n_pair_q) {
          const int t0 = 2 * pr;
          f32x4 sc[2], dp[2];
#pragma unroll
          for (int t = 0; t < 2; ++t) {
            f32x4 dlv = *(const f32x4*)(s_delta + (t0 + t) * 16 + 4 * g);
            for (int w = 1; w < n_t; ++w) dlv += *(const f32x4*)(s_delta + w * rows_img + (t0 + t) * 16 + 4 * g);
#pragma unroll
            for (int r = 0; r < 4; ++r) {
              const float p = pA[pr][t][r];
              dp[t][r] = p * (dA[pr][t][r] - dlv[r]);
              sc[t][r] = (keepA[pr] >> (4 * t + r)) & 1u ? p : 0.f;
            }
          }
          const bf16x8 fp = v2_pack(sc[0], sc[1]);
          const bf16x8 fs = v2_pack(dp[0], dp[1]);
          onepass_put_ds(ds_row + t0 * 16, fs, t0 + 1 < n_tq);
#pragma unroll
          for (int d = 0; d < ND; ++d) {
            dv[d] = mfma_bf16(v2_frag_tr<HD>(img1, t0, d * 16, lane), fp, dv[d]);
            dk[d] = mfma_bf16(v2_frag_tr<HD>(img0, t0, d * 16, lane), fs, dk[d]);
          }
        }
      }
    }
    for (int pr = 0; pr < (EXACT ? 0 : n_pair_q); ++pr) {
      const int t0 = 2 * pr;
      f32x4 sc[2], dp[2];
#pragma unroll
      for (int t = 0; t < 2; ++t) { sc[t] = f32x4{0.f, 0.f, 0.f, 0.f}; dp[t] = f32x4{0.f, 0.f, 0.f, 0.f}; }
#pragma unroll
      for (int t = 0; t < 2; ++t)
#pragma unroll
        for (int ks = 0; ks < v2_ks<HD>; ++ks) {
          sc[t] = mfma_bf16(v2_frag_lds<HD>(img0, (t0 + t) * 16, ks * 32, lane), fk[ks], sc[t]);
          dp[t] = mfma_bf16(v2_frag_lds<HD>(img1, (t0 + t) * 16, ks * 32, lane), fv[ks], dp[t]);
        }
      __builtin_amdgcn_sched_barrier(0);
#pragma unroll
      for (int t = 0; t < 2; ++t) {
        const int qb = (t0 + t) * 16 + 4 * g;
        const f32x4 l2v = *(const f32x4*)(s_lse + qb);
        const f32x4 dlv = *(const f32x4*)(s_delta + qb);
        bool keep[4] = {true, true, true, true};
        if constexpr (DROP) attn_keep4_queries(P.drop, kh, qb, s2h, odd, keep);
        v2_p_ds<false>(sc[t], dp[t], scale2, kb, l2v, dlv, keep);
      }
      const bf16x8 fp = v2_pack(sc[0], sc[1]);
      const bf16x8 fs = v2_pack(dp[0], dp[1]);
      onepass_put_ds(ds_row + t0 * 16, fs, t0 + 1 < n_tq);
#pragma unroll
      for (int d = 0; d < ND; ++d) {
        dv[d] = mfma_bf16(v2_frag_tr<HD>(img1, t0, d * 16, lane), fp, dv[d]);
        dk[d] = mfma_bf16(v2_frag_tr<HD>(img0, t0, d * 16, lane), fs, dk[d]);
      }
      __builtin_amdgcn_sched_barrier(0);
    }
    static_assert(ND == 4, "rows4_exchange: 64-column rows");
    const Row32 kv = rows4_exchange(dk, a.scale * ik), vv = rows4_exchange(dv, ik);
    if (kok) {
      rows4_store(dqkv + (int64_t)key * gld + D, kv, g);
      rows4_store(dqkv + (int64_t)key * gld + 2 * D, vv, g);
    }
  } else if constexpr (EXACT) {
    __syncthreads();
  }
  __syncthreads();
  if (kt < n_t) onepass_put_k<HD>(img0, fk, kt, lane);
  __syncthreads();
  for (int qt = wave; qt < n_tq; qt += nw) {
    const int q = qt * 16 + c;
    f32x4 dq[ND];
#pragma unroll
    for (int d = 0; d < ND; ++d) dq[d] = f32x4{0.f, 0.f, 0.f, 0.f};
    for (int pk = 0; pk < n_pair_k; ++pk) {
      const bf16x8 fs = v2_frag_tr_ld(dsT, ldq, 2 * pk, qt * 16, lane, 2 * pk + 1 < n_t);
#pragma unroll
      for (int d = 0; d < ND; ++d) dq[d] = mfma_bf16(v2_frag_tr<HD>(img0, 2 * pk, d * 16, lane), fs, dq[d]);
    }
    const Row32 qv = rows4_exchange(dq, a.scale * ik);
    if (q < S) rows4_store(dqkv + (int64_t)q * gld, qv, g);
  }
}

template <int HD, bool DROP>
__global__ __launch_bounds__(1024) __attribute__((amdgpu_waves_per_eu(4, 4))) void attn_bwd_v4_kernel(AttnParams P, int rows_img, int ldq) {
  attn_bwd_v4_body<HD, DROP, false>(P, rows_img, ldq);
}
template <int HD, bool DROP>
__global__ __launch_bounds__(512) void attn_bwd_v4x_kernel(AttnParams P, int rows_img, int ldq) {
  attn_bwd_v4_body<HD, DROP, true>(P, rows_img, ldq);
}

template <int HD, bool DROP, int NU>
__device__ __forceinline__ void v5_phase1(const AttnParams& P, const bf16_t* img0, const bf16_t* img1, const float* s_kb, const float* s_lse,
                                          const float* s_delta, bf16_t* dsT, int ldq, const bf16x8 (&wk)[2][v2_ks<HD>], const bf16x8 (&wv)[2][v2_ks<HD>],
                                          int wave, int lane, int S, int SL, int drop_bh, int n_tq, bf16_t* dqkv, int64_t gld, int D, float ik) {
  constexpr int ND = HD / 16;
  const mdt_attn_fwd_args& a = P.f;
  const int g = lane >> 4, c = lane & 15, odd = c & 1;
  const uint32_t s2h = (uint32_t)((SL + 1) >> 1);
  const float scale2 = a.scale * LOG2E;
  const uint32_t base_rp = (uint32_t)(drop_bh * SL) * s2h;
  const int n_pair_q = (n_tq + 1) >> 1;
  int key[NU];
  float kb[NU];
  uint32_t kh[NU];
  bf16_t* ds_row[NU];
  f32x4 dv[NU][ND], dk[NU][ND];
#pragma unroll
  for (int u = 0; u < NU; ++u) {
    key[u] = (wave + 8 * u) * 16 + c;
    kb[u] = s_kb[key[u]];
    kh[u] = base_rp + (uint32_t)(key[u] >> 1);
    ds_row[u] = dsT + key[u] * ldq + 4 * g;
#pragma unroll
    for (int d = 0; d < ND; ++d) { dv[u][d] = f32x4{0.f, 0.f, 0.f, 0.f}; dk[u][d] = f32x4{0.f, 0.f, 0.f, 0.f}; }
  }
  for (int pr = 0; pr < n_pair_q; ++pr) {
    const int t0 = 2 * pr;
    f32x4 sc[NU][2], dp[NU][2];
#pragma unroll
    for (int u = 0; u < NU; ++u)
#pragma unroll
      for (int t = 0; t < 2; ++t) { sc[u][t] = f32x4{0.f, 0.f, 0.f, 0.f}; dp[u][t] = f32x4{0.f, 0.f, 0.f, 0.f}; }
#pragma unroll
    for (int t = 0; t < 2; ++t)
#pragma unroll
      for (int ks = 0; ks < v2_ks<HD>; ++ks) {
        const bf16x8 aq = v2_frag_lds<HD>(img0, (t0 + t) * 16, ks * 32, lane), ao = v2_frag_lds<HD>(img1, (t0 + t) * 16, ks * 32, lane);
#pragma unroll
        for (int u = 0; u < NU; ++u) {
          sc[u][t] = mfma_bf16(aq, wk[u][ks], sc[u][t]);
          dp[u][t] = mfma_bf16(ao, wv[u][ks], dp[u][t]);
        }
      }
    bf16x8 fp[NU], fs[NU];
    {
      f32x4 l2v[2], dlv[2];
#pragma unroll
      for (int t = 0; t < 2; ++t) {
        const int qb = (t0 + t) * 16 + 4 * g;
        l2v[t] = *(const f32x4*)(s_lse + qb);
        dlv[t] = *(const f32x4*)(s_delta + qb);
      }
#pragma unroll
      for (int u = 0; u < NU; ++u) {
#pragma unroll
        for (int t = 0; t < 2; ++t) {
          const int qb = (t0 + t) * 16 + 4 * g;
          bool keep[4] = {true, true, true, true};
          if constexpr (DROP) attn_keep4_queries(P.drop, kh[u], qb, s2h, odd, keep);
          v2_p_ds<false>(sc[u][t], dp[u][t], scale2, kb[u], l2v[t], dlv[t], keep);
        }
        fp[u] = v2_pack(sc[u][0], sc[u][1]);
        fs[u] = v2_pack(dp[u][0], dp[u][1]);
        onepass_put_ds(ds_row[u] + t0 * 16, fs[u], t0 + 1 < n_tq);
      }
    }
#pragma unroll
    for (int d = 0; d < ND; ++d) {
      const bf16x8 to = v2_frag_tr<HD>(img1, t0, d * 16, lane), tq = v2_frag_tr<HD>(img0, t0, d * 16, lane);
#pragma unroll
      for (int u = 0; u < NU; ++u) {
        dv[u][d] = mfma_bf16(to, fp[u], dv[u][d]);
        dk[u][d] = mfma_bf16(tq, fs[u], dk[u][d]);
      }
    }
  }
  static_assert(ND == 4, "rows4_exchange: 64-column rows");
#pragma unroll
  for (int u = 0; u < NU; ++u) {
    const Row32 kv = rows4_exchange(dk[u], a.scale * ik), vv = rows4_exchange(dv[u], ik);
    if (key[u] < S) {
      rows4_store(dqkv + (int64_t)key[u] * gld + D, kv, g);
      rows4_store(dqkv + (int64_t)key[u] * gld + 2 * D, vv, g);
    }
  }
}

__device__ __forceinline__ int v5_opaque(int x) {
  asm volatile("" : "+v"(x));
  return x;
}
__device__ __forceinline__ int v5_sload(const int* p) {
  int v;
  asm volatile("s_load_dword %0, %1, 0x0\n\ts_waitcnt lgkmcnt(0)" : "=s"(v) : "s"(p));
  return v;
}

template <int HD, bool DROP>
__global__ __launch_bounds__(512) __attribute__((amdgpu_waves_per_eu(2, 2))) void attn_bwd_v5_kernel(AttnParams P, int rows_img, int ldq, int n_items) {
  constexpr int NCH = 4;
  extern __shared__ __attribute__((aligned(16))) char smem[];
  const mdt_attn_fwd_args& a = P.f;
  const int tid = threadIdx.x, lane = tid & 63, wave = __builtin_amdgcn_readfirstlane(tid >> 6);
  const int SL = a.S, D = a.H * HD;
  const int64_t tld = a.pos_stride * a.ld_qkv, dld = a.pos_stride * P.ld_dout, old_ = a.pos_stride * a.ld_out, gld = a.pos_stride * P.ld_dqkv;
  bf16_t* img0 = (bf16_t*)smem;
  bf16_t* img1 = img0 + rows_img * v2_ld<HD>;
  float* s_kb = (float*)(img1 + rows_img * v2_ld<HD>);
  float* s_lse = s_kb + rows_img;
  float* s_delta = s_lse + rows_img;
  bf16_t* dsT = (bf16_t*)(s_delta + rows_img);
  const float ik = DROP ? P.drop.inv_keep : 1.0f, rik = 1.0f / ik;

  int seq, h, S, n_t, rows_live, q_rows;
  int64_t row0;
  auto item_of = [&](int it_) {
    const int it = __builtin_amdgcn_readfirstlane(it_);
    const int si = it / a.H;
    h = it - si * a.H;
    seq = a.seq_ids ? v5_sload(a.seq_ids + si) : si;
    if (a.seq_offsets) {
      const int o0 = v5_sload(a.seq_offsets + seq), o1 = v5_sload(a.seq_offsets + seq + 1);
      S = o1 - o0;
      row0 = o0;
    } else {
      S = a.S;
      row0 = (int64_t)seq * a.seq_stride;
    }
    n_t = (S + 15) >> 4;
    rows_live = ((n_t + 1) >> 1) * 32;
    if (rows_live > rows_img || S <= 0) { S = 0; n_t = 0; rows_live = 0; }
    q_rows = (a.q_limit > 0 && ((a.q_limit + 15) & ~15) < S) ? ((a.q_limit + 15) & ~15) : S;
  };
  bf16x8 cq[NCH], cg[NCH], co[NCH];
  float lv = 0.f;
  KeyBytes kbv{1, 0};
  bf16x8 wk[2][v2_ks<HD>], wv[2][v2_ks<HD>];
  auto request_rows = [&](int tid) {
    if (S > 0) {
      const bf16_t* qkv = (const bf16_t*)a.qkv + row0 * a.ld_qkv + h * HD;
      const bf16_t* dout = (const bf16_t*)P.dout + row0 * P.ld_dout + h * HD;
      const bf16_t* outp = (const bf16_t*)a.out + row0 * a.ld_out + h * HD;
      onepass_request<HD, NCH, true>(cq, cg, co, lv, kbv, a, bias_ctx(a, seq, h, S), qkv, dout, outp, tld, dld, old_, SL, q_rows, rows_live, tid, 512);
    }
  };
  auto request_frags = [&](int tid) {
    if (S > 0) {
      const int lane = tid & 63, wave = tid >> 6;
      const bf16_t* qkv = (const bf16_t*)a.qkv + row0 * a.ld_qkv + h * HD;

#pragma unroll
      for (int u = 0; u < 2; ++u)
#pragma unroll
        for (int ks = 0; ks < v2_ks<HD>; ++ks) {
          wk[u][ks] = v2_frag_glb<HD>(qkv + D, tld, S, (wave + 8 * u) * 16, ks * 32, lane);
          wv[u][ks] = v2_frag_glb<HD>(qkv + 2 * D, tld, S, (wave + 8 * u) * 16, ks * 32, lane);
        }
    }
  };

  int it = blockIdx.x;
  if (it >= n_items) return;
  item_of(it);
  request_rows(tid);
  request_frags(tid);
  for (;;) {
    const int cS = S, c_nt = n_t, c_rows = rows_live, c_qrows = q_rows, c_seq = seq, c_h = h;
    const int64_t c_row0 = row0;
    const int tid1 = v5_opaque(tid);
    onepass_stage<HD, NCH>(img0, img1, s_kb, s_lse, s_delta, cq, cg, co, lv, kbv, bias_ctx(a, c_seq, c_h, cS), c_qrows, c_rows, rik, tid1, 512);
#pragma unroll
    for (int u = 0; u < 2; ++u)
#pragma unroll
      for (int ks = 0; ks < v2_ks<HD>; ++ks) asm volatile("" ::"v"(wk[u][ks]), "v"(wv[u][ks]));
    __syncthreads();
    const int nxt = it + (int)gridDim.x;
    const bool more = nxt < n_items;
    if (more) { item_of(nxt); request_rows(v5_opaque(tid)); }
    bf16_t* dqkv = (bf16_t*)P.dqkv + c_row0 * P.ld_dqkv + c_h * HD;
    const int n_tq = (a.q_limit > 0 && ((a.q_limit + 15) >> 4) < c_nt) ? (a.q_limit + 15) >> 4 : c_nt;
    const int lane1 = v5_opaque(lane);
    if (wave + 8 < c_nt) v5_phase1<HD, DROP, 2>(P, img0, img1, s_kb, s_lse, s_delta, dsT, ldq, wk, wv, wave, lane1, cS, SL, c_seq * a.H + c_h, n_tq, dqkv, gld, D, ik);
    else if (wave < c_nt) v5_phase1<HD, DROP, 1>(P, img0, img1, s_kb, s_lse, s_delta, dsT, ldq, wk, wv, wave, lane1, cS, SL, c_seq * a.H + c_h, n_tq, dqkv, gld, D, ik);
    __syncthreads();
    const int tid2 = v5_opaque(tid), lane2 = tid2 & 63;
#pragma unroll
    for (int u = 0; u < 2; ++u)
      if (wave + 8 * u < c_nt) onepass_put_k<HD>(img0, wk[u], wave + 8 * u, lane2);
    if (more) request_frags(tid2);
    __syncthreads();
    onepass_phase2<HD>(img0, dsT, ldq, dqkv, gld, cS, c_nt, n_tq, wave, 8, v5_opaque(lane), a.scale * ik);
    if (!more) break;
    it = nxt;
    __syncthreads();
  }
}

template <bool DROP>
static int launch_one_pass(hipStream_t st, const AttnParams& p, const AttnPlan& pl) {
  const dim3 grid(p.f.H, p.f.nseq);
  const size_t lds = attn_one_pass_lds_bytes(pl.n_t);
  if (pl.route == AttnRoute::v5) return launch_route<attn_bwd_v5_kernel<64, DROP>>("v5", dim3((unsigned)pl.wgs), 512, lds, st, p, pl.rows_img, pl.ldq, pl.items);
  if (pl.route == AttnRoute::v4x) return launch_route<attn_bwd_v4x_kernel<64, DROP>>("v4x", grid, pl.waves * 64, lds, st, p, pl.rows_img, pl.ldq);
  return launch_route<attn_bwd_v4_kernel<64, DROP>>("v4", grid, pl.waves * 64, lds, st, p, pl.rows_img, pl.ldq);
}

template <int HD, bool STRUCT, bool DROP>
static int launch_v3(hipStream_t st, const AttnParams& p, const AttnPlan& pl) {
  if constexpr (HD == 64 && !STRUCT) {
    if (pl.route != AttnRoute::v3) return launch_one_pass<DROP>(st, p, pl);
  }
  const size_t lds = attn_v3_lds_bytes(HD, pl.s_pad, pl.tight, pl.nhist);
  const dim3 grid(p.f.H, p.f.nseq);
  if constexpr (HD > 64) {
    if (pl.tight) return launch_route<attn_bwd_v3_tight_kernel<HD, STRUCT, DROP>>("v3", grid, pl.threads, lds, st, p, pl.s_pad);
    return launch_route<attn_bwd_v3_kernel<HD, STRUCT, DROP>>("v3", grid, pl.threads, lds, st, p, pl.s_pad);
  } else if constexpr (STRUCT) return launch_route<attn_bwd_v3_kernel<HD, true, DROP>>("v3", grid, pl.threads, lds, st, p, pl.s_pad);
  else return launch_route<attn_bwd_v3_occ4_kernel<HD, DROP>>("v3", grid, pl.threads, lds, st, p, pl.s_pad);
}

template <int HD, int NT, bool STRUCT, bool DROP, bool BWD>
static int launch_v2(hipStream_t st, const AttnParams& p, const AttnPlan& pl) {
  const size_t lds = attn_v2_lds_bytes(HD, NT, BWD, pl.nhist);
  const dim3 grid(p.f.H, p.f.nseq);
  if constexpr (BWD && NT > 7) return attn_unplanned("the v2 backward past 112 keys");
  else if constexpr (BWD) return launch_route<attn_bwd_v2_kernel<HD, NT, STRUCT, DROP>>("v2", grid, 256, lds, st, p);
  else {
    constexpr int NWF = attn_v2_fwd_waves(NT, STRUCT);
    return launch_route<attn_fwd_v2_kernel<HD, NT, STRUCT, DROP, NWF>>("v2", grid, NWF * 64, lds, st, p);
  }
}

int attention_v2_launch(hipStream_t st, const AttnParams& p, const AttnPlan& pl) {
  return with_head_dim(p.f.hd, [&](auto hd) { return with_flags(pl, [&](auto s, auto d) {
    constexpr int HD = decltype(hd)::value;
    constexpr bool STRUCT = decltype(s)::value, DROP = decltype(d)::value;
    if (pl.route != AttnRoute::v2) return launch_v3<HD, STRUCT, DROP>(st, p, pl);
    return with_rung<2, 4, 5, 7, 9, 13, 17>(pl.rung, [&](auto nt) {
      constexpr int NT = decltype(nt)::value;
      return pl.bwd ? launch_v2<HD, NT, STRUCT, DROP, true>(st, p, pl) : launch_v2<HD, NT, STRUCT, DROP, false>(st, p, pl);
    });
  }); });
}

}
```

multimodaldiscussiontransformer_amd/engine.py:

```python
from __future__ import annotations

import os

import contextlib
import threading
import weakref
from dataclasses import dataclass
from typing import Callable, List, Optional, Sequence

import torch

from . import fp8 as F8
from . import ops


_DETERMINISTIC = os.environ.get("MDT_DETERMINISTIC", "0") == "1"


def set_deterministic(on: bool) -> None:
    global _DETERMINISTIC
    if on and F8.ACTIVE is not None:
        raise NotImplementedError("deterministic mode with fp8 GEMMs: the fp8 path has no ordered reductions (disable fp8 first)")
    _DETERMINISTIC = bool(on)

# ... 152 lines not shown
        finally:
            self._leave_side()
            self.record(self._enter_side)

    def _crossing(self, v: "Var", t: torch.Tensor):
        if self.side is not None and v.side != _SS.side_active:
            t.record_stream(self.side if v.side else self._main)

    def next_seed(self) -> int:
        if self._seed_base is None:
            self._seed_base = int(torch.randint(0, 2 ** 62, (1,)).item())
        self._seed_ctr += 1
        return (self._seed_base + 0x9E3779B97F4A7C15 * self._seed_ctr) & 0x7FFFFFFFFFFFFFFF

    def record(self, bwd: Callable[[], None]):
        if not self.inference:
            self.ops.append(bwd)

    def adjoint(self, o: "Var", bwd: Callable[[torch.Tensor], None], take: bool = True):
        def run():
            g = o.grad
            if take:
                o.grad = None
            if g is not None:
                bwd(g)

        self.record(run)

    def pgrad(self, p: torch.nn.Parameter) -> Optional[torch.Tensor]:
        if p is None or not p.requires_grad:
            return None
        if self.use_main_grad:
            g = getattr(p, "main_grad", None)
            if g is None:
                raise RuntimeError("use_main_grad=True but a trainable parameter has no .main_grad buffer")
            return g
        g = self.tmp_grads.get(id(p))
        if g is None:
            g = torch.zeros(p.shape, dtype=torch.float32, device=p.device)
            self.tmp_grads[id(p)] = g
        return g

    def grad_buf(self, v: Var) -> torch.Tensor:
        if v.grad is None:
            if self.side is not None and v.side and not _SS.side_active:
                with torch.cuda.stream(self.side):
                    v.grad = torch.zeros_like(v.data)
                torch.cuda.current_stream().wait_stream(self.side)
            else:
                v.grad = torch.zeros_like(v.data)
                self._crossing(v, v.grad)
        return v.grad

    def add_grad(self, v: Var, g: torch.Tensor):
        if not v.needs_grad:
            return
        if v.grad is None:
            v.grad = g
            self._crossing(v, g)
        else:
            ops.row_axpby(v.grad, v.grad.shape[0], a=g, accumulate=True)

    def backward(self):
        try:
            while self.ops:
                self.ops.pop()()
        finally:
            self._leave_side()
        self.ops = []
        self.sync_streams()
        if F8.ACTIVE is not None:
            F8.ACTIVE.end_of_step()

    def sync_streams(self):
        if self.side is not None:
            torch.cuda.current_stream().wait_stream(self.side)


@dataclass
class LoraSlot:
    A: torch.nn.Parameter
    Bt: torch.nn.Parameter
    scale: float = 1.0


@dataclass
class BlockParams:
    qkv_w: torch.nn.Parameter
    qkv_b: torch.nn.Parameter
    o_w: torch.nn.Parameter
    o_b: torch.nn.Parameter
    ln1_w: torch.nn.Parameter
    ln1_b: torch.nn.Parameter
    fc1_w: torch.nn.Parameter
    fc1_b: torch.nn.Parameter
    fc2_w: torch.nn.Parameter
    fc2_b: torch.nn.Parameter
    ln2_w: torch.nn.Parameter
    ln2_b: torch.nn.Parameter
    lora_A: Optional[torch.nn.Parameter] = None
    lora_Bt: Optional[torch.nn.Parameter] = None
    lora_cols: Optional[tuple] = None
    lora_scale: float = 1.0
    lora_o: Optional[LoraSlot] = None
    lora_fc1: Optional[LoraSlot] = None
    lora_fc2: Optional[LoraSlot] = None

    def dense_lora(self):
        return [s for s in (self.lora_o, self.lora_fc1, self.lora_fc2) if s is not None]

    def all(self):
        base = [self.qkv_w, self.qkv_b, self.o_w, self.o_b, self.ln1_w, self.ln1_b, self.fc1_w, self.fc1_b,
                self.fc2_w, self.fc2_b, self.ln2_w, self.ln2_b]
        if self.lora_A is not None:
            base = base + [self.lora_A, self.lora_Bt]
        return base + [p for s in self.dense_lora() for p in (s.A, s.Bt)]


@dataclass
class AttnSpec:
    nseq: int
    S: int
    H: int
    seq_stride: Optional[int] = None
    pos_stride: int = 1
    scale: Optional[float] = None
    key_mask: Optional[torch.Tensor] = None
    dense_bias: Optional[torch.Tensor] = None
    dense_bias_var: Optional[Var] = None
    attn_bias: Optional[torch.Tensor] = None
    spatial_pos: Optional[torch.Tensor] = None
    sp_table: Optional[torch.nn.Parameter] = None
    virt: Optional[torch.nn.Parameter] = None
    key_pad: Optional[torch.Tensor] = None
    seq_offsets: Optional[torch.Tensor] = None
    q_limit: int = 0
    bins: Optional[list] = None

    def kwargs(self):
        return dict(seq_stride=self.seq_stride, pos_stride=self.pos_stride, scale=self.scale, key_mask=self.key_mask,
                    seq_offsets=self.seq_offsets, q_limit=self.q_limit, bins=self.bins,
                    dense_bias=self.dense_bias, attn_bias=self.attn_bias, spatial_pos=self.spatial_pos,
                    sp_table=None if self.sp_table is None else self.sp_table.data,
                    virt=None if self.virt is None else self.virt.data.view(-1), key_pad=self.key_pad)


def _split_k(n_out: int, k_out: int, red: int) -> int:
    tiles = ((n_out + 127) // 128) * ((k_out + 127) // 128)
    s = max(1, 1024 // max(1, tiles))
    return int(max(1, min(s, red // 1024 if red >= 1024 else 1)))


_WGRAD_ASUM = os.environ.get("MDT_WGRAD_ASUM", "1") != "0"


def wgrad(tape: Tape, dy: torch.Tensor, x: torch.Tensor, w: torch.nn.Parameter, b: Optional[torch.nn.Parameter]):
    gw = tape.pgrad(w)
    gb = tape.pgrad(b) if b is not None else None
    if gw is not None:
        ride = gb is not None and dy.dtype == torch.bfloat16 and _WGRAD_ASUM and not _DETERMINISTIC
        wgrad_gemm(dy, x, gw.view(dy.shape[1], x.shape[1]), asum=gb.view(-1) if ride else None)
        if ride:
            return
    if gb is not None:
        colsum(dy, out=gb.view(-1))


_LN_BIAS_RIDE = os.environ.get("MDT_LN_BIAS_RIDE", "1") != "0"


EMBED_LN_FUSED = os.environ.get("MDT_EMBED_LN_FUSED", "1") != "0"
PATCH_K_PAD = os.environ.get("MDT_PATCH_K_PAD", "1") != "0"
PATCH_EMBED_FUSED = os.environ.get("MDT_PATCH_EMBED_FUSED", "1") != "0"
WEIGHT_EPOCH = 0


def weights_changed():
    global WEIGHT_EPOCH
    WEIGHT_EPOCH += 1


def weight_stamp(w: torch.nn.Parameter) -> tuple:
    return (w._version, WEIGHT_EPOCH, w.data_ptr())


_KP_CACHE: dict = {}


def _k_padded(w: torch.nn.Parameter, wmat: torch.Tensor, kp: int) -> torch.Tensor:
    key = (id(w), kp)
    ver = weight_stamp(w)
    hit = _KP_CACHE.get(key)
    if hit is not None and hit[0]() is w and hit[1] == ver:
        return hit[2]
    wp = torch.zeros(wmat.shape[0], kp, dtype=wmat.dtype, device=wmat.device)
    wp[:, :wmat.shape[1]].copy_(wmat)
    _KP_CACHE[key] = (weakref.ref(w), ver, wp)
    return wp


def dgrad(dy: torch.Tensor, w: torch.nn.Parameter, **kw) -> torch.Tensor:
    return ops.gemm(dy, w.data, trans_b=True, **kw)


def linear(f8, x: torch.Tensor, w: torch.nn.Parameter, tag: str, *, grad=False, x8=None, q8_site=None, q8_grad=False, **kw):
    r = None if f8 is None else f8.linear(x, w, (tag, id(w)), transposed_weight=grad, grad=grad, x8=x8, q8_site=q8_site,
                                          q8_grad=q8_grad, **kw)
    if r is None:
        return (dgrad(x, w, **kw) if grad else ops.gemm(x, w.data, **kw)), None
    return r if q8_site is not None else (r, None)


def dyd_rides(g: torch.Tensor) -> bool:
    return _LN_BIAS_RIDE and g.dtype == torch.bfloat16 and g.shape[0] >= 8192 and not _DETERMINISTIC


def _ln_bwd(tape, dy, x, w, b, mean, rstd, add=None):
    return layernorm_bwd(dy, x, w.data, mean, rstd, add=add, dgamma=tape.pgrad(w), dbeta=tape.pgrad(b))


def _ln_bwd_dense(tape, dy, x, w, b, mean, rstd, bias_param, p_drop, seed, add=None):
    gb = tape.pgrad(bias_param) if bias_param is not None else None
    return layernorm_bwd(dy, x, w.data, mean, rstd, add=add, dgamma=tape.pgrad(w), dbeta=tape.pgrad(b),
                         drop_p=p_drop, drop_seed=seed, colsum=None if gb is None else gb.view(-1),
                         want_dropped=True)


def lora_fwd(P: BlockParams, src: torch.Tensor, qkv: torch.Tensor) -> torch.Tensor:
    D = src.shape[1]
    r = P.lora_A.shape[0] // len(P.lora_cols)
    t = ops.lora_down(src, P.lora_A.data)
    for j, c in enumerate(P.lora_cols):
        ops.lora_up_add(t[:, j * r:(j + 1) * r], P.lora_Bt.data[j * r:(j + 1) * r], qkv[:, c * D:(c + 1) * D], alpha=P.lora_scale)
    return t


def lora_bwd(tape: Tape, P: BlockParams, src: torch.Tensor, t: torch.Tensor, dqkv: torch.Tensor, dx: Optional[torch.Tensor]) -> None:
    D = src.shape[1]
    n = P.lora_A.shape[0]
    r = n // len(P.lora_cols)
    s = P.lora_scale
    gA, gBt = tape.pgrad(P.lora_A), tape.pgrad(P.lora_Bt)
    want_dt = gA is not None or dx is not None
    dt = torch.empty(src.shape[0], n, dtype=src.dtype, device=src.device) if want_dt else None
    ws = None
    if gA is not None or gBt is not None:
        ws = ordered_workspace(ops.lib.mdt_lora_wgrad_workspace_bytes(src.shape[0], n, D), src.device)
    for j, c in enumerate(P.lora_cols):
        rows, dq = slice(j * r, (j + 1) * r), dqkv[:, c * D:(c + 1) * D]
        if gBt is not None:
            ops.lora_wgrad(t[:, rows], dq, gBt.view(n, D)[rows], alpha=s, ws=ws)
        if want_dt:
            ops.lora_down(dq, P.lora_Bt.data[rows], out=dt[:, rows], alpha=s)
    if gA is not None:
        ops.lora_wgrad(dt, src, gA.view(n, D), ws=ws)
    if dx is not None:
        ops.lora_up_add(dt, P.lora_A.data, dx)


def lora_dense_bwd(tape: Tape, L: LoraSlot, src: torch.Tensor, t: torch.Tensor, g: torch.Tensor, dx: Optional[torch.Tensor]) -> torch.Tensor:
    r = L.A.shape[0]
    gA, gBt = tape.pgrad(L.A), tape.pgrad(L.Bt)
    ws = None
    if gA is not None or gBt is not None:
        wide = max(src.shape[1], g.shape[1])
        ws = ordered_workspace(ops.lib.mdt_lora_wgrad_workspace_bytes(src.shape[0], r, wide), src.device)
    if gBt is not None:
        ops.lora_wgrad(t, g, gBt.view(r, g.shape[1]), alpha=L.scale, ws=ws)
    dt = ops.lora_down(g, L.Bt.data, alpha=L.scale)
    if gA is not None:
        ops.lora_wgrad(dt, src, gA.view(r, src.shape[1]), ws=ws)
    if dx is not None:
        ops.lora_up_add(dt, L.A.data, dx)
    return dt


def transformer_block(tape: Tape, x: Var, P: BlockParams, spec: AttnSpec, *, pre_ln: bool, eps: float,
                      p_hidden: float = 0.0, p_attn: float = 0.0, p_act: float = 0.0, keep_rows=None, act: str = "gelu",
                      recompute: str = "none") -> Var:
    xd = x.data
    s_attn, s_o, s_act, s_f2 = (tape.next_seed() for _ in range(4))
    kw = dict(spec.kwargs(), drop_p=p_attn, drop_seed=s_attn)
    R = None if keep_rows is None else int(keep_rows.numel())
    f8 = F8.ACTIVE
    if act not in ops.ACT_KINDS:
        raise ValueError(f"transformer_block: unknown activation {act!r} (one of {sorted(ops.ACT_KINDS)})")
    if act != "gelu" and f8 is not None:
        raise NotImplementedError(f"fp8 GEMMs with the {act} activation: the fused fp8 producer of h is fc1's erf-GELU epilogue")
    if P.lora_A is not None and f8 is not None:
        raise NotImplementedError("fp8 GEMMs on a block with low-rank adapters: the adapter sum enters the bf16 qkv buffer only "
                                  "(run adapters in bf16, or fp8 without --lora-rank)")
    Lo, L1, L2 = P.lora_o, P.lora_fc1, P.lora_fc2
    if P.dense_lora() and f8 is not None:
        raise NotImplementedError("fp8 GEMMs on a block with low-rank adapters: the adapter sums of the output projection, fc1 and "
                                  "fc2 enter bf16 buffers only (run adapters in bf16, or fp8 without --lora-rank)")
    policy = "none" if tape.inference else _checked_policy(recompute)
    if policy != "none" and f8 is not None:
        raise NotImplementedError(f"transformer_block(recompute={policy!r}) with fp8 GEMMs: {RECOMPUTE_FP8_WHY}")

    def gather(src):
        if keep_rows is None:
            return src
        out_ = torch.empty(R, src.shape[1], dtype=src.dtype, device=src.device)
        ops.row_axpby(out_, R, a=src, ai=keep_rows)
        return out_

    def spread(g_):
        if keep_rows is None:
            return g_
        full = torch.zeros(xd.shape[0], g_.shape[1], dtype=g_.dtype, device=g_.device)
        ops.row_axpby(full, R, di=keep_rows, a=g_)
        return full

    def ln8(x_, lw, lb, w_, tag):
        slot = None if (f8 is None or x_.dtype != torch.bfloat16) else f8.producer_slot(x_.shape[0], w_, (tag, id(w_)))
        if slot is None:
            return (*ops.layernorm_fwd(x_, lw.data, lb.data, eps), None)
        return (*ops.layernorm_fwd(x_, lw.data, lb.data, eps, q8=slot[:4]), (slot[0], slot[4]))

    def run():
        def attn_fwd(src, src8):
            qkv_, _ = linear(f8, src, P.qkv_w, "qkv", x8=src8, bias=P.qkv_b.data)
            lt_ = None
            if P.lora_A is not None:
                lt_ = lora_fwd(P, src, qkv_)
                if tape.inference:
                    lt_ = None
            ctx_full_, lse_ = ops.attention_fwd(qkv_, spec.nseq, spec.S, spec.H, **kw)
            ctx_, xk = gather(ctx_full_), gather(xd)
            t_ = ops.gemm(ctx_, P.o_w.data, bias=P.o_b.data, residual=xk, drop_p=p_hidden, drop_seed=s_o)
            if Lo is not None:
                lto = ops.lora_down(ctx_, Lo.A.data)
                ops.lora_up_add_drop(lto, Lo.Bt.data, t_, alpha=Lo.scale, drop_p=p_hidden, drop_seed=s_o)
                if not tape.inference:
                    lts["o"] = lto
            return qkv_, lt_, ctx_full_, lse_, ctx_, t_

        def fc2_fwd(h_, h8, res):
            y_ = linear(f8, h_, P.fc2_w, "fc2", x8=h8, bias=P.fc2_b.data, residual=res, drop_p=p_hidden, drop_seed=s_f2)[0]
            if L2 is not None:
                lt2 = ops.lora_down(h_, L2.A.data)
                ops.lora_up_add_drop(lt2, L2.Bt.data, y_, alpha=L2.scale, drop_p=p_hidden, drop_seed=s_f2)
                if not tape.inference:
                    lts["fc2"] = lt2
            return y_

        def fc1_fwd(src, src8):
            if L1 is not None:
                pre_ = ops.gemm(src, P.fc1_w.data, bias=P.fc1_b.data)
                lt1 = ops.lora_down(src, L1.A.data)
                h_, u_ = ops.lora_up_act(lt1, L1.Bt.data, pre_, act, alpha=L1.scale, drop_p=p_act, drop_seed=s_act, out=pre_,
                                         want_u=not tape.inference)
                if not tape.inference:
                    lts["fc1"] = lt1
                return u_, h_, None
            if act != "gelu":
                pre_ = ops.gemm(src, P.fc1_w.data, bias=P.fc1_b.data)
                h_, u_ = ops.act_fwd(pre_, act, drop_p=p_act, drop_seed=s_act, out=pre_, want_u=not tape.inference)
                return u_, h_, None
            u_ = torch.empty(src.shape[0], P.fc1_w.shape[0], dtype=src.dtype, device=src.device)
            h_, h8 = linear(f8, src, P.fc1_w, "fc1", x8=src8, q8_site=("fc2", id(P.fc2_w)), bias=P.fc1_b.data, aux=u_,
                            epilogue=ops.EPI_GELU | ops.EPI_AUX_GRAD, drop_p=p_act, drop_seed=s_act)
            return u_, h_, h8

        def ffn_fwd(src, src8, res):
            u_, h_, h8 = fc1_fwd(src, src8)
            return u_, h_, fc2_fwd(h_, h8, res)

        lts = {}
        if not pre_ln:
            a_in = xd
            qkv, lt, ctx_full, lse, ctx, t = attn_fwd(a_in, None)
            f_in, m1, r1, f_in8 = ln8(t, P.ln1_w, P.ln1_b, P.fc1_w, "fc1")
            u, h, y = ffn_fwd(f_in, f_in8, f_in)
            out, m2, r2 = ops.layernorm_fwd(y, P.ln2_w.data, P.ln2_b.data, eps)
        else:
            a_in, m1, r1, a_in8 = ln8(xd, P.ln1_w, P.ln1_b, P.qkv_w, "qkv")
            qkv, lt, ctx_full, lse, ctx, t = attn_fwd(a_in, a_in8)
            f_in, m2, r2, f_in8 = ln8(t, P.ln2_w, P.ln2_b, P.fc1_w, "fc1")
            u, h, out = ffn_fwd(f_in, f_in8, t)
        if policy == "ffn":
            u = h = None
            lts.pop("fc1", None)
            lts.pop("fc2", None)

        def ffn_bwd(gd, fc2_b, dres):
            nonlocal u, h
            if policy == "ffn":
                u, h, _ = fc1_fwd(f_in, None)
                if L2 is not None:
                    lts["fc2"] = ops.lora_down(h, L2.A.data)
            wgrad(tape, gd, h, P.fc2_w, fc2_b)
            gb1 = tape.pgrad(P.fc1_b)
            det = _DETERMINISTIC
            late = det or L2 is not None
            dt2 = lora_dense_bwd(tape, L2, h, lts["fc2"], gd, None) if L2 is not None else None
            du, du8 = linear(f8, gd, P.fc2_w, "d_fc2", grad=True, q8_site=("d_fc1", id(P.fc1_w)), q8_grad=True, aux=u,
                             epilogue=ops.EPI_MULAUX, colsum=None if (gb1 is None or late) else gb1.view(-1))
            if L2 is not None:
                ops.lora_up_add_mul(dt2, L2.A.data, du, u)
            if late and gb1 is not None:
                colsum(du, out=gb1.view(-1))
            wgrad(tape, du, f_in, P.fc1_w, None)
            df = linear(f8, du, P.fc1_w, "d_fc1", grad=True, x8=du8, residual=dres)[0]
            if L1 is not None:
                lora_dense_bwd(tape, L1, f_in, lts["fc1"], du, df)
            if policy == "ffn":
                u = h = None
            return df

        def attn_bwd(dtd, o_b, want_dx, dres=None):
            wgrad(tape, dtd, ctx, P.o_w, o_b)
            dctx = ops.gemm(dtd, P.o_w.data, trans_b=True)
            if Lo is not None:
                lora_dense_bwd(tape, Lo, ctx, lts["o"], dtd, dctx)
            dqkv = _attention_bwd(tape, spec, kw, dctx, qkv, ctx_full, lse, spread)
            wgrad(tape, dqkv, a_in, P.qkv_w, P.qkv_b)
            dx_ = dgrad(dqkv, P.qkv_w, residual=None if dres is None else spread(dres)) if want_dx else None
            if P.lora_A is not None:
                lora_bwd(tape, P, a_in, lt, dqkv, dx_)
            return dx_

        def bwd(g):
            ride = _WGRAD_ASUM and dyd_rides(g)
            if not pre_ln:
                dy, dyd = _ln_bwd_dense(tape, g, y, P.ln2_w, P.ln2_b, m2, r2, None if ride else P.fc2_b, p_hidden, s_f2)
                df = ffn_bwd(dyd, P.fc2_b if ride else None, dy)
                dt_, dtd = _ln_bwd_dense(tape, df, t, P.ln1_w, P.ln1_b, m1, r1, None if ride else P.o_b, p_hidden, s_o)
                dx = attn_bwd(dtd, P.o_b if ride else None, x.needs_grad, dt_)
                if x.needs_grad:
                    tape.add_grad(x, dx)
            else:
                gd = ops.dropout(g, p_hidden, s_f2) if p_hidden > 0 else g
                df = ffn_bwd(gd, P.fc2_b, None)
                dt_, dtd = _ln_bwd_dense(tape, df, t, P.ln2_w, P.ln2_b, m2, r2, None if ride else P.o_b, p_hidden, s_o, add=g)
                da = attn_bwd(dtd, P.o_b if ride else None, True)
                if x.needs_grad:
                    tape.add_grad(x, _ln_bwd(tape, da, xd, P.ln1_w, P.ln1_b, m1, r1, add=spread(dt_)))
                else:
                    _ln_bwd(tape, da, xd, P.ln1_w, P.ln1_b, m1, r1)
            if tape.on_params_ready:
                tape.on_params_ready(P.all())

        return out, bwd

    if policy == "block":
        out = run()[0]

        def bwd(g):
            replayed = run()[1]
            replayed(g)
    else:
        out, bwd = run()
    o = Var(out)
    tape.adjoint(o, bwd)
    return o


def _attention_bwd(tape: Tape, spec: AttnSpec, kw: dict, dctx, qkv, ctx, lse, spread=lambda g: g):
    extra = {}
    if spec.sp_table is not None and _DETERMINISTIC:
        return _attention_bwd_ordered(tape, spec, kw, dctx, qkv, ctx, lse, spread)
    if spec.sp_table is not None:
        extra = dict(d_sp_table=tape.pgrad(spec.sp_table),
                     d_virt=None if tape.pgrad(spec.virt) is None else tape.pgrad(spec.virt).view(-1))
    want_dense = spec.dense_bias_var is not None and spec.dense_bias_var.needs_grad
    dqkv, dbias = ops.attention_bwd(spread(dctx), qkv, ctx, lse, spec.nseq, spec.S, spec.H, **kw, want_dense_dbias=want_dense,
                                    **extra)
    if want_dense:
        tape.add_grad(spec.dense_bias_var, dbias)
    return dqkv


def _attention_bwd_ordered(tape: Tape, spec: AttnSpec, kw: dict, dctx, qkv, ctx, lse, spread):
    if spec.S > 272:
        raise NotImplementedError(f"deterministic mode: a structural attention bias over {spec.S} tokens takes the long path "
                                  "(S > 272), whose bias gradient exists with float atomics only")
    dqkv, dS = ops.attention_bwd(spread(dctx), qkv, ctx, lse, spec.nseq, spec.S, spec.H, **kw, want_dense_dbias=True)
    gt, gv = tape.pgrad(spec.sp_table), tape.pgrad(spec.virt)
    if gt is not None:
        ws = ordered_workspace(ops.lib.mdt_attn_bias_grad_ordered_workspace_bytes(spec.nseq, spec.H, gt.shape[0]), dS.device)
        ops.attn_bias_grad_ordered(dS, spec.spatial_pos, gt, None if gv is None else gv.view(-1), ws=ws)
    if spec.dense_bias_var is not None and spec.dense_bias_var.needs_grad:
        tape.add_grad(spec.dense_bias_var, dS)
    return dqkv


def attention_layer(tape: Tape, x: Var, qkv_w, qkv_b, o_w, o_b, spec: AttnSpec, p_attn: float = 0.0, stash: Optional[dict] = None) -> Var:
    xd = x.data
    kw = dict(spec.kwargs(), drop_p=p_attn, drop_seed=tape.next_seed())
    qkv = ops.gemm(xd, qkv_w.data, bias=None if qkv_b is None else qkv_b.data)
    ctx, lse = ops.attention_fwd(qkv, spec.nseq, spec.S, spec.H, **kw)
    if stash is not None:
        stash.update(qkv=qkv, lse=lse, kw=spec.kwargs())
    out = ops.gemm(ctx, o_w.data, bias=None if o_b is None else o_b.data)
    o = Var(out)

    def bwd(g):
        wgrad(tape, g, ctx, o_w, o_b)
        dqkv = _attention_bwd(tape, spec, kw, ops.gemm(g, o_w.data, trans_b=True), qkv, ctx, lse)
        wgrad(tape, dqkv, xd, qkv_w, qkv_b)
        if x.needs_grad:
            tape.add_grad(x, ops.gemm(dqkv, qkv_w.data, trans_b=True))

    tape.adjoint(o, bwd)
    return o


def layernorm(tape: Tape, x: Var, w, b, eps: float) -> Var:
    y, mean, rstd = ops.layernorm_fwd(x.data, w.data, b.data, eps)
    o = Var(y)

    def bwd(g):
        dx = _ln_bwd(tape, g, x.data, w, b, mean, rstd)
        tape.add_grad(x, dx)

    tape.adjoint(o, bwd)
    return o


def dropout(tape: Tape, x: Var, p: float) -> Var:
    if p <= 0.0:
        return x
    seed = tape.next_seed()
    o = Var(ops.dropout(x.data, p, seed))

    def bwd(g):
        tape.add_grad(x, ops.dropout(g, p, seed))

    tape.adjoint(o, bwd)
    return o


def bert_embeddings(tape: Tape, ids, types, word, pos, typ) -> Var:
    M, Lq = ids.shape
    D = word.shape[1]
    out = torch.empty(M * Lq, D, dtype=word.dtype, device=word.device)
    ops.bert_embed_sum(ids, types, word.data, pos.data, typ.data, out, out_seq_stride=Lq, out_off=0)
    o = Var(out)

    def bwd(g):
        gw, gp = tape.pgrad(word), tape.pgrad(pos)
        if gw is not None:
            scatter_add(gw, ids.view(-1), g, M * Lq)
        if gp is not None:
            colsum(g.view(M, Lq * D), out=gp[:Lq].view(-1))
        _type_emb_grad(tape, g, types.view(-1), typ)

    tape.adjoint(o, bwd)
    return o


def _type_emb_grad(tape: Tape, g, types, typ):
    gt = tape.pgrad(typ)
    if gt is None:
        return
    assert typ.shape[0] == 2, "token-type gradient is implemented for type_vocab_size == 2"
    D = g.shape[1]
    tot = colsum(g)
    one = colsum(g, row_weight=types)
    ops.row_axpby(gt, 1, d_off=1, a=one.view(1, D), accumulate=True)
    ops.row_axpby(gt, 1, d_off=0, a=tot.view(1, D), b=one.view(1, D), beta=-1.0, accumulate=True)


def _embed_rows_grads(tape: Tape, g, rows, ids, types, pos_ids, word, pos, typ):
    gw, gp = tape.pgrad(word), tape.pgrad(pos)
    if gw is not None:
        scatter_add(gw, ids, g, rows)
    if gp is not None:
        scatter_add(gp, pos_ids, g, rows)
    _type_emb_grad(tape, g, types, typ)


def bert_embeddings_rows(tape: Tape, ids, types, pos_ids, word, pos, typ) -> Var:
    rows = ids.numel()
    D = word.shape[1]
    out = torch.empty(rows, D, dtype=word.dtype, device=word.device)
    ops.bert_embed_rows(ids, types, pos_ids, word.data, pos.data, typ.data, out)
    o = Var(out)

    def bwd(g):
        _embed_rows_grads(tape, g, rows, ids, types, pos_ids, word, pos, typ)

    tape.adjoint(o, bwd)
    return o


def bert_embeddings_ln_rows(tape: Tape, ids, types, pos_ids, word, pos, typ, w, b, eps: float) -> Var:
    rows = ids.numel()
    y, mean, rstd, xs = ops.bert_embed_ln_rows(ids, types, pos_ids, word.data, pos.data, typ.data, w.data, b.data, eps,
                                               keep_sum=not tape.inference)
    o = Var(y)

    def bwd(g):
        dx = _ln_bwd(tape, g, xs, w, b, mean, rstd)
        _embed_rows_grads(tape, dx, rows, ids, types, pos_ids, word, pos, typ)

    tape.adjoint(o, bwd)
    return o


def vit_embeddings(tape: Tape, images, proj_w, proj_b, cls, pos, patch: int) -> Var:
    I = images.shape[0]
    D = proj_w.shape[0]
    g_ = images.shape[-1] // patch
    npatch = g_ * g_
    wmat = proj_w.data.view(D, -1)
    tokens = torch.empty(I * (npatch + 1), D, dtype=proj_w.dtype, device=proj_w.device)
    fused = (PATCH_EMBED_FUSED and proj_w.dtype == torch.bfloat16 and patch == 16 and D % 128 == 0
             and (tape.inference or not (proj_w.requires_grad or proj_b.requires_grad)))
    cols = patches = None
    if fused:
        ops.vit_patch_embed(images, patch, wmat, proj_b.data, cls.data.view(-1), pos.data.view(npatch + 1, D), tokens,
                            seq_stride=npatch + 1, off=0)
    else:
        kin = wmat.shape[1]
        kp = kin if (kin % 128 == 0 or proj_w.dtype != torch.bfloat16 or not PATCH_K_PAD) else (kin + 127) // 128 * 128
        cols = ops.vit_patchify(images, patch, proj_w.dtype, k_pad=kp)
        patches = ops.gemm(cols, _k_padded(proj_w, wmat, kp) if kp != kin else wmat, bias=proj_b.data)
        ops.vit_assemble(patches, cls.data.view(-1), pos.data.view(npatch + 1, D), tokens, I, npatch,
                         seq_stride=npatch + 1, off=0)
# ... 232 lines not shown
```

multimodaldiscussiontransformer_amd/ops.py:

```python
from __future__ import annotations

import ctypes as C
from typing import Optional

import torch

from . import _lib as L
from ._lib import (EPI_ACCUM, EPI_ASUM, EPI_ATOMIC, EPI_AUX_GRAD, EPI_BIAS, EPI_COLSUM, EPI_DGELU, EPI_DROPOUT, EPI_GELU, EPI_MULAUX, EPI_RESIDUAL, check, dt, lib,
                   ptr, stream)
from ._lib import ACT_GELU, ACT_GELU_ACCURATE, ACT_LINEAR, ACT_RELU, ACT_TANH, MdtError

__all__ = [
    "bert_embed_rows",
    "gemm", "colsum", "layernorm_fwd", "layernorm_bwd", "attention_fwd", "attention_bwd", "attention_mean_probs", "graph_attn_bias",
    "row_axpby", "row_scatter_add", "bert_embed_sum", "bert_embed_ln_rows", "vit_patchify", "vit_assemble", "vit_patch_embed", "graph_node_feature",
    "tanh_fwd", "tanh_bwd", "node_ce", "contrastive_loss", "fp8_quantize", "fp8_scale_update", "gemm_fp8", "cast", "transpose2d", "dropout", "dropout_mask",
    "sum_slices", "gemm_splitk_ordered", "colsum_ordered", "layernorm_bwd_ordered", "segments_of", "row_segment_sum",
    "attn_bias_grad_ordered", "float_atomic_launches", "lora_down", "lora_up_add", "lora_up_add_drop", "lora_up_add_mul", "lora_up_act", "lora_wgrad",
    "LORA_WGRAD_SLAB",
    "act_fwd", "ACT_KINDS", "ACT_GELU", "ACT_RELU", "ACT_GELU_ACCURATE", "ACT_TANH", "ACT_LINEAR",
    "EPI_BIAS", "EPI_GELU", "EPI_RESIDUAL", "EPI_DGELU", "EPI_ACCUM", "EPI_ATOMIC", "EPI_DROPOUT", "EPI_AUX_GRAD", "EPI_MULAUX", "EPI_ASUM",
]


def _2d(t: torch.Tensor):
    assert t.dim() == 2 and t.stride(1) == 1, "expected a row-major 2-D tensor (unit inner stride)"
    return t.stride(0)


def gemm(a: torch.Tensor, b: torch.Tensor, *, trans_a=False, trans_b=False, out: Optional[torch.Tensor] = None,
         out_dtype=None, bias=None, residual=None, aux=None, epilogue=0, alpha=1.0, split_k=1, drop_p=0.0,
         drop_seed=0, colsum=None, asum=None) -> torch.Tensor:
    lda, ldb = _2d(a), _2d(b)
    M, K = (a.shape[1], a.shape[0]) if trans_a else (a.shape[0], a.shape[1])
    N = b.shape[1] if trans_b else b.shape[0]
    kb = b.shape[0] if trans_b else b.shape[1]
    assert kb == K, f"gemm: inner dimensions differ ({K} vs {kb})"
    assert a.dtype == b.dtype
    if out is None:
        out = torch.empty(M, N, dtype=out_dtype or a.dtype, device=a.device)
    assert out.shape == (M, N)
    if bias is not None:
        epilogue |= EPI_BIAS
        assert bias.dtype == a.dtype and bias.numel() == N and bias.is_contiguous()
    if residual is not None:
        epilogue |= EPI_RESIDUAL
        assert residual.dtype == a.dtype and residual.shape == (M, N)
    if aux is not None:
        assert aux.dtype == a.dtype and aux.shape == (M, N)
    if drop_p > 0.0:
        epilogue |= EPI_DROPOUT
    if colsum is not None:
        epilogue |= EPI_COLSUM
        assert colsum.dtype == torch.float32 and colsum.numel() == N
    if asum is not None:
        assert colsum is None and trans_a and asum.dtype == torch.float32 and asum.numel() == M and asum.is_contiguous()
        epilogue |= EPI_ASUM
        colsum = asum
    check(lib.mdt_gemm(stream(), dt(a), dt(out), int(trans_a), int(trans_b), M, N, K, ptr(a), lda, ptr(b), ldb,
                       ptr(out), _2d(out), epilogue, float(alpha), ptr(bias), ptr(residual),
                       _2d(residual) if residual is not None else 0, ptr(aux), _2d(aux) if aux is not None else 0,
                       int(split_k), float(drop_p), int(drop_seed), ptr(colsum)), "mdt_gemm")
    return out


def colsum(x: torch.Tensor, out: Optional[torch.Tensor] = None, row_weight=None) -> torch.Tensor:
    if out is None:
        out = torch.zeros(x.shape[1], dtype=torch.float32, device=x.device)
    assert row_weight is None or (row_weight.dtype == torch.int32 and row_weight.numel() == x.shape[0])
    check(lib.mdt_colsum(stream(), dt(x), x.shape[0], x.shape[1], ptr(x), _2d(x), ptr(out), ptr(row_weight)),
          "mdt_colsum")
    return out


def layernorm_fwd(x, gamma, beta, eps, out=None, q8=None):
    rows, D = x.shape
    if out is None:
        out = torch.empty_like(x)
    mean = torch.empty(rows, dtype=torch.float32, device=x.device)
    rstd = torch.empty(rows, dtype=torch.float32, device=x.device)
    if q8 is not None:
        q8_out, q8_format, q8_scale, q8_amax = q8
        assert q8_out.dtype == torch.uint8 and q8_out.shape == (rows, D)
        check(lib.mdt_layernorm_fwd_q8(stream(), dt(x), rows, D, ptr(x), _2d(x), ptr(gamma), ptr(beta), float(eps), ptr(out), _2d(out),
                                       ptr(mean), ptr(rstd), ptr(q8_out), _2d(q8_out), int(q8_format), ptr(q8_scale), ptr(q8_amax)),
              "mdt_layernorm_fwd_q8")
        return out, mean, rstd
    check(lib.mdt_layernorm_fwd(stream(), dt(x), rows, D, ptr(x), _2d(x), ptr(gamma), ptr(beta), float(eps), ptr(out),
                                _2d(out), ptr(mean), ptr(rstd)), "mdt_layernorm_fwd")
    return out, mean, rstd


def layernorm_bwd(dy, x, gamma, mean, rstd, add=None, dgamma=None, dbeta=None, dx=None, drop_p=0.0, drop_seed=0,
                  colsum=None, want_dropped=False):
    rows, D = x.shape
    if dx is None:
        dx = torch.empty_like(x)
    dxd = torch.empty_like(x) if (want_dropped and drop_p > 0.0) else None
    check(lib.mdt_layernorm_bwd(stream(), dt(x), rows, D, ptr(dy), _2d(dy), ptr(x), _2d(x), ptr(gamma), ptr(mean),
                                ptr(rstd), ptr(add), _2d(add) if add is not None else 0, ptr(dx), _2d(dx),
                                ptr(dgamma), ptr(dbeta), ptr(dxd), _2d(dxd) if dxd is not None else 0, float(drop_p),
                                int(drop_seed), ptr(colsum)), "mdt_layernorm_bwd")
    if want_dropped:
        return dx, (dxd if dxd is not None else dx)
    return dx


def _attn_args(qkv, out, lse, nseq, S, H, hd, seq_stride, pos_stride, scale, key_mask, dense_bias, attn_bias,
               spatial_pos, sp_table, virt, key_pad, drop_p=0.0, drop_seed=0, seq_offsets=None, q_limit=0, seq_ids=None, s_cap=0):
    hd = qkv.shape[1] // 3 // H if hd is None else hd
    seq_stride = S if seq_stride is None else seq_stride
    scale = hd ** -0.5 if scale is None else scale
    a = L.AttnFwdArgs()
    a.q_limit = int(q_limit)
    a.drop_p, a.drop_seed = float(drop_p), int(drop_seed)
    assert seq_offsets is None or (seq_offsets.dtype == torch.int32 and seq_offsets.is_contiguous() and
                                   seq_offsets.numel() == nseq + 1), "attention: seq_offsets must be i32[nseq + 1]"
    a.seq_offsets = ptr(seq_offsets)
    a.dtype = dt(qkv)
    a.nseq, a.S, a.H, a.hd = nseq, S, H, hd
    a.s_cap = int(s_cap)
    if seq_ids is not None:
        assert seq_offsets is not None and seq_ids.dtype == torch.int32 and seq_ids.is_contiguous()
        a.seq_ids, a.nseq, a.nseq_total = ptr(seq_ids), int(seq_ids.numel()), nseq
    a.seq_stride, a.pos_stride, a.scale = seq_stride, pos_stride, float(scale)
    a.qkv, a.ld_qkv = ptr(qkv), _2d(qkv)
    a.out, a.ld_out = ptr(out), _2d(out)
    a.lse = ptr(lse)
    a.key_mask = ptr(key_mask)
    a.dense_bias = ptr(dense_bias)
    a.attn_bias = ptr(attn_bias)
    a.spatial_pos = ptr(spatial_pos)
    a.sp_table = ptr(sp_table)
    a.virt = ptr(virt)
    a.key_pad = ptr(key_pad)
    a.num_spatial = sp_table.shape[0] if sp_table is not None else 0
    for t, want in ((key_mask, torch.uint8), (key_pad, torch.uint8), (dense_bias, torch.float32),
                    (attn_bias, torch.float32), (spatial_pos, torch.int32)):
        assert t is None or (t.dtype == want and t.is_contiguous()), f"attention: expected contiguous {want}"
    return a


def _attn_bins(bins, qkv, H, S):
    if bins is None or qkv.dtype != torch.bfloat16 or qkv.shape[1] // 3 // H != 64 or S > 272:
        return [(None, 0)]
    return [(ids, cap) for ids, cap in bins if ids.numel() > 0]


def _f32_out(out, shape, device):
    if out is None:
        return torch.empty(shape, dtype=torch.float32, device=device)
    assert out.shape == tuple(shape) and out.dtype == torch.float32 and out.is_contiguous(), f"expected contiguous f32{list(shape)}"
    return out


def attention_route(args, bwd):
    name, geo = C.create_string_buffer(16), (C.c_int32 * 2)()
    check(lib.mdt_attention_route(C.byref(args), int(bool(bwd)), name, len(name), geo), "mdt_attention_route")
    return name.value.decode(), (geo[0], geo[1])


def attention_fwd(qkv, nseq, S, H, *, seq_stride=None, pos_stride=1, scale=None, key_mask=None, dense_bias=None,
                  attn_bias=None, spatial_pos=None, sp_table=None, virt=None, key_pad=None, drop_p=0.0, drop_seed=0,
                  seq_offsets=None, q_limit=0, bins=None, out=None, lse=None):
    D = qkv.shape[1] // 3
    if out is None:
        out = torch.empty(qkv.shape[0], D, dtype=qkv.dtype, device=qkv.device)
    if lse is None:
        lse = torch.empty(nseq, H, S, dtype=torch.float32, device=qkv.device)
    assert out.shape == (qkv.shape[0], D) and out.dtype == qkv.dtype, "attention_fwd: out must be [rows, D] of qkv's type"
    assert lse.shape == (nseq, H, S) and lse.dtype == torch.float32 and lse.is_contiguous(), "attention_fwd: lse must be contiguous f32[nseq, H, S]"
    for ids, cap in _attn_bins(bins, qkv, H, S):
        a = _attn_args(qkv, out, lse, nseq, S, H, None, seq_stride, pos_stride, scale, key_mask, dense_bias, attn_bias, spatial_pos,
                       sp_table, virt, key_pad, drop_p, drop_seed, seq_offsets, q_limit, ids, cap)
        check(lib.mdt_attention_fwd(stream(), C.byref(a)), "mdt_attention_fwd")
    return out, lse


def attention_mean_probs(qkv, lse, nseq, S, H, *, seq_stride=None, pos_stride=1, scale=None, key_mask=None, dense_bias=None,
                         attn_bias=None, spatial_pos=None, sp_table=None, virt=None, key_pad=None, out=None):
    out = _f32_out(out, (nseq, S, S), qkv.device)
    a = _attn_args(qkv, qkv, lse, nseq, S, H, None, seq_stride, pos_stride, scale, key_mask, dense_bias, attn_bias, spatial_pos, sp_table,
                   virt, key_pad)
    check(lib.mdt_attention_mean_probs(stream(), C.byref(a), ptr(out)), "mdt_attention_mean_probs")
    return out


def attention_head_weights(qkv, lse, nseq, S, H, *, raw_scores=False, seq_stride=None, pos_stride=1, scale=None, key_mask=None,
                           dense_bias=None, attn_bias=None, spatial_pos=None, sp_table=None, virt=None, key_pad=None, out=None):
    out = _f32_out(out, (nseq, H, S, S), qkv.device)
    if lse is None:
        assert raw_scores
        lse = torch.empty(nseq * H * S, dtype=torch.float32, device=qkv.device)
    a = _attn_args(qkv, qkv, lse, nseq, S, H, None, seq_stride, pos_stride, scale, key_mask, dense_bias, attn_bias, spatial_pos, sp_table,
                   virt, key_pad)
    check(lib.mdt_attention_head_weights(stream(), C.byref(a), 1 if raw_scores else 0, ptr(out)), "mdt_attention_head_weights")
    return out


def attention_bwd(dout, qkv, out, lse, nseq, S, H, *, seq_stride=None, pos_stride=1, scale=None, key_mask=None,
                  dense_bias=None, attn_bias=None, spatial_pos=None, sp_table=None, virt=None, key_pad=None,
                  want_dense_dbias=False, d_sp_table=None, d_virt=None, drop_p=0.0, drop_seed=0, seq_offsets=None, q_limit=0,
                  bins=None, dqkv=None, dbias=None):
    D = qkv.shape[1] // 3
    if dqkv is None:
        dqkv = torch.empty(qkv.shape, dtype=qkv.dtype, device=qkv.device)
    assert dqkv.shape == qkv.shape and dqkv.dtype == qkv.dtype, "attention_bwd: dqkv must have qkv's shape and type"
    if q_limit:
        dqkv[:, :D].zero_()
    if dbias is not None:
        dbias = _f32_out(dbias, (nseq, H, S, S), qkv.device).zero_()
    elif want_dense_dbias:
        dbias = torch.zeros(nseq, H, S, S, dtype=torch.float32, device=qkv.device)
    for ids, cap in _attn_bins(bins, qkv, H, S):
        b = L.AttnBwdArgs()
        b.f = _attn_args(qkv, out, lse, nseq, S, H, None, seq_stride, pos_stride, scale, key_mask, dense_bias, attn_bias, spatial_pos,
                         sp_table, virt, key_pad, drop_p, drop_seed, seq_offsets, q_limit, ids, cap)
        b.dout, b.ld_dout = ptr(dout), _2d(dout)
        b.dqkv, b.ld_dqkv = ptr(dqkv), _2d(dqkv)
        b.d_dense_bias = ptr(dbias)
        b.d_sp_table = ptr(d_sp_table)
        b.d_virt = ptr(d_virt)
        check(lib.mdt_attention_bwd(stream(), C.byref(b)), "mdt_attention_bwd")
    return dqkv, dbias


def graph_attn_bias(attn_bias, spatial_pos, sp_table, virt, out=None):
    nseq, S, _ = attn_bias.shape
    H = sp_table.shape[1]
    out = _f32_out(out, (nseq, H, S, S), attn_bias.device)
    check(lib.mdt_graph_attn_bias(stream(), dt(sp_table), nseq, S, H, ptr(attn_bias), ptr(spatial_pos), ptr(sp_table),
                                  ptr(virt), ptr(out)), "mdt_graph_attn_bias")
    return out


def row_axpby(dst, nrows, *, di=None, d_inner=1, d_stride=1, d_off=0, a=None, ai=None, a_inner=1, a_stride=1, a_off=0,
              alpha=1.0, b=None, bi=None, b_inner=1, b_stride=1, b_off=0, beta=1.0, accumulate=False):
    D = dst.shape[1]
    for t in (di, ai, bi):
        assert t is None or (t.dtype == torch.int32 and t.is_contiguous())
    check(lib.mdt_row_axpby(stream(), dt(dst), nrows, D, ptr(dst), _2d(dst), ptr(di), d_inner, d_stride, d_off,
                            ptr(a), _2d(a) if a is not None else 0, ptr(ai), a_inner, a_stride, a_off, float(alpha),
                            ptr(b), _2d(b) if b is not None else 0, ptr(bi), b_inner, b_stride, b_off, float(beta),
                            int(accumulate)), "mdt_row_axpby")
    return dst


def row_scatter_add(table_f32, idx, src, nrows, *, s_stride=1, s_off=0):
    assert table_f32.dtype == torch.float32 and idx.dtype == torch.int32
    check(lib.mdt_row_scatter_add_f32(stream(), dt(src), nrows, table_f32.shape[1], ptr(table_f32), _2d(table_f32),
                                      ptr(idx), ptr(src), _2d(src), s_stride, s_off), "mdt_row_scatter_add_f32")
    return table_f32


def _workspace(ws, need: int, device):
    if ws is None:
        ws = torch.empty(max(int(need), 16), dtype=torch.uint8, device=device)
    assert ws.dtype == torch.uint8 and ws.is_contiguous()
    return ws, ws.numel()


def float_atomic_launches(reset: bool = False) -> int:
    return int(lib.mdt_float_atomic_launches(int(reset)))


def sum_slices(ws: torch.Tensor, out: torch.Tensor, accumulate: bool = False) -> torch.Tensor:
    assert ws.dim() == 3 and out.dim() == 2 and ws.shape[1:] == out.shape and ws.dtype == out.dtype == torch.float32
    assert ws.shape[2] == 0 or (ws.stride(2) == 1 and out.stride(1) == 1)
    check(lib.mdt_sum_slices_f32(stream(), out.shape[0], out.shape[1], ws.shape[0], ptr(ws), ws.stride(1), ws.stride(0), ptr(out),
                                 out.stride(0), int(accumulate)), "mdt_sum_slices_f32")
    return out


def gemm_splitk_ordered(a: torch.Tensor, b: torch.Tensor, out: torch.Tensor, *, trans_a=False, trans_b=False, alpha=1.0,
                        split_k=1, ws=None) -> torch.Tensor:
    lda, ldb = _2d(a), _2d(b)
    M, K = (a.shape[1], a.shape[0]) if trans_a else (a.shape[0], a.shape[1])
    N = b.shape[1] if trans_b else b.shape[0]
    assert (b.shape[0] if trans_b else b.shape[1]) == K and a.dtype == b.dtype
    assert out.dtype == torch.float32 and out.shape == (M, N)
    ws, nbytes = _workspace(ws, lib.mdt_gemm_splitk_ordered_workspace_bytes(M, N, int(split_k)), a.device)
    check(lib.mdt_gemm_splitk_ordered(stream(), dt(a), int(trans_a), int(trans_b), M, N, K, ptr(a), lda, ptr(b), ldb, ptr(out),
                                      _2d(out), float(alpha), int(split_k), ptr(ws), nbytes), "mdt_gemm_splitk_ordered")
    return out


LORA_WGRAD_SLAB = int(lib.mdt_lora_wgrad_slab_rows())


def lora_down(x: torch.Tensor, w: torch.Tensor, out: Optional[torch.Tensor] = None, alpha=1.0) -> torch.Tensor:
    R, K = x.shape
    n = w.shape[0]
    assert w.shape[1] == K and x.dtype == w.dtype
    if out is None:
        out = torch.empty(R, n, dtype=x.dtype, device=x.device)
    assert out.shape == (R, n) and out.dtype == x.dtype
    check(lib.mdt_lora_down(stream(), dt(x), R, n, K, ptr(x), _2d(x), ptr(w), _2d(w), ptr(out), _2d(out), float(alpha)), "mdt_lora_down")
    return out


def lora_up_add(t: torch.Tensor, w: torch.Tensor, y: torch.Tensor, alpha=1.0) -> torch.Tensor:
    R, n = t.shape
    N = w.shape[1]
    assert w.shape[0] == n and y.shape == (R, N) and t.dtype == w.dtype == y.dtype
    check(lib.mdt_lora_up_add(stream(), dt(t), R, n, N, ptr(t), _2d(t), ptr(w), _2d(w), ptr(y), _2d(y), float(alpha)), "mdt_lora_up_add")
    return y


def lora_up_add_drop(t: torch.Tensor, w: torch.Tensor, y: torch.Tensor, alpha=1.0, drop_p=0.0, drop_seed=0) -> torch.Tensor:
    R, n = t.shape
    N = w.shape[1]
    assert w.shape[0] == n and y.shape == (R, N) and t.dtype == w.dtype == y.dtype
    check(lib.mdt_lora_up_add_drop(stream(), dt(t), R, n, N, ptr(t), _2d(t), ptr(w), _2d(w), ptr(y), _2d(y), float(alpha),
                                   float(drop_p), int(drop_seed)), "mdt_lora_up_add_drop")
    return y


def lora_up_add_mul(t: torch.Tensor, w: torch.Tensor, y: torch.Tensor, aux: torch.Tensor, alpha=1.0) -> torch.Tensor:
    R, n = t.shape
    N = w.shape[1]
    assert w.shape[0] == n and y.shape == (R, N) and aux.shape == (R, N) and t.dtype == w.dtype == y.dtype == aux.dtype
    check(lib.mdt_lora_up_add_mul(stream(), dt(t), R, n, N, ptr(t), _2d(t), ptr(w), _2d(w), ptr(y), _2d(y), ptr(aux), _2d(aux),
                                  float(alpha)), "mdt_lora_up_add_mul")
    return y


def lora_up_act(t: torch.Tensor, w: torch.Tensor, pre: torch.Tensor, kind, *, alpha=1.0, drop_p=0.0, drop_seed=0, want_u=True,
                out=None, u=None):
    k = ACT_KINDS[kind] if isinstance(kind, str) else int(kind)
    R, n = t.shape
    N = w.shape[1]
    assert w.shape[0] == n and pre.shape == (R, N) and t.dtype == w.dtype == pre.dtype
    if out is None:
        out = torch.empty_like(pre)
    assert out.dtype == pre.dtype and out.shape == pre.shape
    if u is None and want_u:
        u = torch.empty(pre.shape, dtype=pre.dtype, device=pre.device)
    assert u is None or (u.dtype == pre.dtype and u.shape == pre.shape)
    check(lib.mdt_lora_up_act(stream(), dt(t), k, R, n, N, ptr(t), _2d(t), ptr(w), _2d(w), ptr(pre), _2d(pre), ptr(out), _2d(out),
                              ptr(u), _2d(u) if u is not None else 0, float(alpha), float(drop_p), int(drop_seed)), "mdt_lora_up_act")
    return out, u


def lora_wgrad(t: torch.Tensor, x: torch.Tensor, dw: torch.Tensor, alpha=1.0, ws=None) -> torch.Tensor:
    R, n = t.shape
    N = x.shape[1]
    assert x.shape[0] == R and t.dtype == x.dtype and dw.dtype == torch.float32 and dw.shape == (n, N)
    ws, nbytes = _workspace(ws, lib.mdt_lora_wgrad_workspace_bytes(R, n, N), t.device)
    check(lib.mdt_lora_wgrad(stream(), dt(t), R, n, N, ptr(t), _2d(t), ptr(x), _2d(x), ptr(dw), _2d(dw), float(alpha), ptr(ws), nbytes),
          "mdt_lora_wgrad")
    return dw


def colsum_ordered(x: torch.Tensor, out: Optional[torch.Tensor] = None, row_weight=None, ws=None) -> torch.Tensor:
    if out is None:
        out = torch.zeros(x.shape[1], dtype=torch.float32, device=x.device)
    assert row_weight is None or (row_weight.dtype == torch.int32 and row_weight.numel() == x.shape[0])
    assert out.dtype == torch.float32 and out.is_contiguous() and out.numel() == x.shape[1]
    ws, nbytes = _workspace(ws, lib.mdt_colsum_ordered_workspace_bytes(x.shape[0], x.shape[1]), x.device)
    check(lib.mdt_colsum_ordered(stream(), dt(x), x.shape[0], x.shape[1], ptr(x), _2d(x), ptr(out), ptr(row_weight), ptr(ws), nbytes),
          "mdt_colsum_ordered")
    return out


def layernorm_bwd_ordered(dy, x, gamma, mean, rstd, add=None, dgamma=None, dbeta=None, dx=None, drop_p=0.0, drop_seed=0,
                          colsum=None, want_dropped=False, ws=None):
    rows, D = x.shape
    if dx is None:
        dx = torch.empty_like(x)
    dxd = torch.empty_like(x) if (want_dropped and drop_p > 0.0) else None
# ... 328 lines not shown
```

Before: 16030 comments/s.

## Precompute attention dropout keep bits in forward and reuse them in v5 backward

A new kernel, launched alongside the attention forward, packs per-key dropout keep decisions into 64-bit words per key tile. The v5 backward kernel gains a variant that loads these words and masks P and dP with bitfield extracts, so it no longer rehashes the dropout RNG inside its inner loop. This trades an extra launch, which recomputes the hashes, plus a small buffer held until backward, for cheaper backward ALU work. It is on by default and applies only to bf16, head dim 64, v5-route launches with at most 13 tiles.

Result: no change. 16100 comments/s (median of 6 runs) (+0.4%).

```diff
diff --git a/include/mdt_hip.h b/include/mdt_hip.h
--- a/include/mdt_hip.h
+++ b/include/mdt_hip.h
@@ -93,6 +93,8 @@
   const int32_t* seq_ids;
   int s_cap;
   int nseq_total;
+  const void* keep_bits;
+  size_t keep_bits_bytes;
 } mdt_attn_fwd_args;
 int mdt_attention_fwd(void* stream, const mdt_attn_fwd_args* a);
 
@@ -106,6 +108,8 @@
 } mdt_attn_bwd_args;
 int mdt_attention_bwd(void* stream, const mdt_attn_bwd_args* a);
 int mdt_attention_route(const mdt_attn_bwd_args* a, int bwd, char* route, size_t route_bytes, int32_t geometry[2]);
+size_t mdt_attention_keep_bits_bytes(const mdt_attn_bwd_args* a);
+int mdt_attention_keep_bits(void* stream, const mdt_attn_bwd_args* a, void* bits, size_t bytes);
 int mdt_attention_mean_probs(void* stream, const mdt_attn_fwd_args* a, float* out);
 int mdt_attention_head_weights(void* stream, const mdt_attn_fwd_args* a, int raw_scores, float* out);
 
diff --git a/multimodaldiscussiontransformer_amd/_lib.py b/multimodaldiscussiontransformer_amd/_lib.py
--- a/multimodaldiscussiontransformer_amd/_lib.py
+++ b/multimodaldiscussiontransformer_amd/_lib.py
@@ -26,6 +26,7 @@
         ("sp_table", _vp), ("virt", _vp), ("key_pad", _vp), ("num_spatial", _i),
         ("drop_p", _f), ("drop_seed", C.c_uint64), ("seq_offsets", _vp), ("q_limit", _i),
         ("seq_ids", _vp), ("s_cap", _i), ("nseq_total", _i),
+        ("keep_bits", _vp), ("keep_bits_bytes", C.c_size_t),
     ]
 
 
@@ -57,6 +58,8 @@
     "mdt_attention_fwd": ([_vp, C.POINTER(AttnFwdArgs)], _i),
     "mdt_attention_bwd": ([_vp, C.POINTER(AttnBwdArgs)], _i),
     "mdt_attention_route": ([C.POINTER(AttnBwdArgs), _i, C.c_char_p, C.c_size_t, C.POINTER(C.c_int32)], _i),
+    "mdt_attention_keep_bits_bytes": ([C.POINTER(AttnBwdArgs)], C.c_size_t),
+    "mdt_attention_keep_bits": ([_vp, C.POINTER(AttnBwdArgs), _vp, C.c_size_t], _i),
     "mdt_attention_mean_probs": ([_vp, C.POINTER(AttnFwdArgs), _vp], _i),
     "mdt_attention_head_weights": ([_vp, C.POINTER(AttnFwdArgs), _i, _vp], _i),
     "mdt_graph_attn_bias": ([_vp, _i, _i, _i, _i, _vp, _vp, _vp, _vp, _vp], _i),
diff --git a/multimodaldiscussiontransformer_amd/build.py b/multimodaldiscussiontransformer_amd/build.py
--- a/multimodaldiscussiontransformer_amd/build.py
+++ b/multimodaldiscussiontransformer_amd/build.py
@@ -8,7 +8,7 @@
 HERE = os.path.dirname(os.path.abspath(__file__))
 CSRC = os.path.join(HERE, "csrc")
 OUT = os.path.join(HERE, "libmdt_hip.so")
-SOURCES = ["gemm.hip", "gemm_wgrad.hip", "gemm_f8.hip", "layernorm.hip", "attention.hip", "attention_v2.hip", "attention_long.hip", "rowops.hip", "elementwise.hip", "ordered.hip", "lora.hip", "activation.hip", "patch_embed.hip", "contrastive.hip", "fp8.hip", "optim.hip", "image.hip", "host.cpp"]
+SOURCES = ["gemm.hip", "gemm_wgrad.hip", "gemm_f8.hip", "layernorm.hip", "attention.hip", "attention_v2.hip", "attention_bits.hip", "attention_long.hip", "rowops.hip", "elementwise.hip", "ordered.hip", "lora.hip", "activation.hip", "patch_embed.hip", "contrastive.hip", "fp8.hip", "optim.hip", "image.hip", "host.cpp"]
 FLAGS = ["--offload-arch=gfx950", "-O3", "-fPIC", "-std=c++17", "-Wno-unused-result", "-ffp-contract=off"]
 EXTRA = {"attention.hip": ["-mllvm", "-amdgpu-mfma-vgpr-form=1"], "attention_v2.hip": ["-mllvm", "-amdgpu-mfma-vgpr-form=1"],
          "gemm_wgrad.hip": ["-mllvm", "-amdgpu-mfma-vgpr-form=1"]}
diff --git a/multimodaldiscussiontransformer_amd/csrc/attention.hip b/multimodaldiscussiontransformer_amd/csrc/attention.hip
--- a/multimodaldiscussiontransformer_amd/csrc/attention.hip
+++ b/multimodaldiscussiontransformer_amd/csrc/attention.hip
@@ -647,9 +647,29 @@
   return MDT_OK;
 }
 
+size_t attn_keep_bits_bytes(const AttnParams& p) {
+  const mdt_attn_fwd_args& a = p.f;
+  if (a.dtype != MDT_BF16 || a.hd != 64 || !(a.drop_p > 0.f)) return 0;
+  const AttnPlan pb = attn_plan(p, true);
+  if (pb.status != MDT_OK || pb.route != AttnRoute::v5 || pb.n_t > 13) return 0;
+  return (size_t)a.nseq * a.H * attn_keep_rows(pb.n_t) * 4 * sizeof(uint64_t);
+}
+
+static int check_keep_bits(AttnParams& p, bool bwd) {
+  if (!p.f.keep_bits) return MDT_OK;
+  const size_t want = bwd ? attn_keep_bits_bytes(p) : 0;
+  MDT_CHECK_ARG(want != 0, "attention: keep_bits given, but the kernels of this launch hash their dropout decisions (mdt_attention_keep_bits_bytes is 0)");
+  MDT_CHECK_ARG(p.f.keep_bits_bytes == want && ((uintptr_t)p.f.keep_bits & 15) == 0,
+                "attention: keep_bits must be the 16-byte aligned buffer of %zu bytes mdt_attention_keep_bits filled for this launch (got %zu)", want,
+                p.f.keep_bits_bytes);
+  p.keep_rows = attn_keep_rows(((p.f.s_cap > 0 ? p.f.s_cap : p.f.S) + 15) / 16);
+  return MDT_OK;
+}
+
 static int dispatch(hipStream_t st, const mdt_attn_fwd_args& f, const mdt_attn_bwd_args* b) {
   AttnParams p;
   if (int e = checked_params(f, b, p)) return e;
+  if (int e = check_keep_bits(p, b != nullptr)) return e;
   if (p.d_sp_table || p.d_virt) note_float_atomic_launch();
   const AttnPlan pl = attn_plan(p, b != nullptr);
   if (pl.status != MDT_OK) return pl.status;
@@ -696,6 +716,26 @@
   return MDT_OK;
 }
 
+extern "C" size_t mdt_attention_keep_bits_bytes(const mdt_attn_bwd_args* a) {
+  AttnParams p;
+  if (!a || a->f.nseq <= 0 || checked_params(a->f, a, p) != MDT_OK) return 0;
+  return attn_keep_bits_bytes(p);
+}
+
+extern "C" int mdt_attention_keep_bits(void* stream, const mdt_attn_bwd_args* a, void* bits, size_t bytes) {
+  MDT_CHECK_ARG(a && bits, "attention_keep_bits: null args");
+  AttnParams p;
+  if (int e = checked_params(a->f, a, p)) return e;
+  const int n_t = ((p.f.s_cap > 0 ? p.f.s_cap : p.f.S) + 15) / 16;
+  MDT_CHECK_ARG(a->f.nseq > 0 && p.f.drop_p > 0.f && n_t <= 13, "attention_keep_bits: needs sequences, drop_p > 0 and rows of at most 208 tokens (s_cap, else S)");
+  const size_t want = (size_t)p.f.nseq * p.f.H * attn_keep_rows(n_t) * 4 * sizeof(uint64_t);
+  MDT_CHECK_ARG(bytes == want && ((uintptr_t)bits & 15) == 0, "attention_keep_bits: bits must be 16-byte aligned and %zu bytes (got %zu)", want, bytes);
+  p.f.keep_bits = bits;
+  p.f.keep_bits_bytes = bytes;
+  p.keep_rows = attn_keep_rows(((p.f.s_cap > 0 ? p.f.s_cap : p.f.S) + 15) / 16);
+  return attention_keep_bits_launch((hipStream_t)stream, p);
+}
+
 extern "C" int mdt_attention_mean_probs(void* stream, const mdt_attn_fwd_args* a, float* out) {
   MDT_CHECK_ARG(a && out, "attention_mean_probs: null args");
   if (a->nseq == 0) return MDT_OK;
diff --git a/multimodaldiscussiontransformer_amd/csrc/attention_bits.hip b/multimodaldiscussiontransformer_amd/csrc/attention_bits.hip
--- /dev/null
+++ b/multimodaldiscussiontransformer_amd/csrc/attention_bits.hip
@@ -0,0 +1,39 @@
+#include "attention_common.hpp"
+
+namespace mdt {
+
+constexpr int KEEP_BITS_WAVES = 4, KEEP_BITS_MAX_TILES = 13;
+__global__ __launch_bounds__(KEEP_BITS_WAVES * 64) void attn_keep_bits_kernel(AttnParams P) {
+  const mdt_attn_fwd_args& a = P.f;
+  const int tid = threadIdx.x, lane = tid & 63, wave = tid >> 6;
+  const int h = blockIdx.x, seq = a.seq_ids ? a.seq_ids[blockIdx.y] : (int)blockIdx.y;
+  const int SL = a.S;
+  const int S = a.seq_offsets ? a.seq_offsets[seq + 1] - a.seq_offsets[seq] : a.S;
+  if (S <= 0 || S > P.keep_rows) return;
+  const int ntk = (S + 15) >> 4;
+  int n_tq = ntk;
+  if (a.q_limit > 0 && ((a.q_limit + 15) >> 4) < n_tq) n_tq = (a.q_limit + 15) >> 4;
+  uint64_t* item = (uint64_t*)a.keep_bits + ((int64_t)blockIdx.y * a.H + h) * (4 * P.keep_rows);
+  const int g = lane >> 4, c = lane & 15, odd = c & 1;
+  const uint32_t s2h = (uint32_t)((SL + 1) >> 1);
+  const uint32_t base_rp = (uint32_t)((seq * a.H + h) * SL) * s2h;
+  for (int kt = wave; kt < ntk; kt += KEEP_BITS_WAVES) {
+    const int key = kt * 16 + c;
+    const uint32_t kh = base_rp + (uint32_t)(key >> 1);
+    uint64_t w = 0;
+    for (int t = 0; t < n_tq; ++t) {
+      bool keep[4];
+      attn_keep4_queries(P.drop, kh, t * 16 + 4 * g, s2h, odd, keep);
+      w |= (uint64_t)((uint32_t)keep[0] | (uint32_t)keep[1] << 1 | (uint32_t)keep[2] << 2 | (uint32_t)keep[3] << 3) << (4 * t);
+    }
+    item[key * 4 + g] = w;
+  }
+}
+
+int attention_keep_bits_launch(hipStream_t st, const AttnParams& p) {
+  if (p.keep_rows > 16 * KEEP_BITS_MAX_TILES) return attn_unplanned("dropout bits for rows of more than 13 key tiles");
+  hipLaunchKernelGGL(attn_keep_bits_kernel, dim3(p.f.H, p.f.nseq), dim3(KEEP_BITS_WAVES * 64), 0, st, p);
+  return check_launch("attention_keep_bits");
+}
+
+}
diff --git a/multimodaldiscussiontransformer_amd/csrc/attention_common.hpp b/multimodaldiscussiontransformer_amd/csrc/attention_common.hpp
--- a/multimodaldiscussiontransformer_amd/csrc/attention_common.hpp
+++ b/multimodaldiscussiontransformer_amd/csrc/attention_common.hpp
@@ -9,6 +9,7 @@
   const void* dout; int64_t ld_dout;
   void* dqkv; int64_t ld_dqkv;
   float* d_dense_bias; float* d_sp_table; float* d_virt;
+  int keep_rows;
 };
 
 struct BiasCtx {
@@ -94,6 +95,9 @@
   const uint32_t w[4] = {odd ? pa : wa, odd ? pb : wb, odd ? wa : pa, odd ? wb : pb};
 #pragma unroll
   for (int r = 0; r < 4; ++r) keep[r] = ((w[r] >> (16 * odd)) & 0xFFFFu) >= d.thresh;
+}
+__device__ __forceinline__ const uint64_t* attn_keep_item(const AttnParams& P, int item) {
+  return (const uint64_t*)P.f.keep_bits + (int64_t)item * (4 * P.keep_rows);
 }
 __device__ __forceinline__ float attn_drop_scale(const DropCfg& d, int bh, int S, int q, int key) {
   const uint32_t w = attn_drop_word(d, attn_row_pairs(bh, S, q), key);
@@ -174,6 +178,9 @@
 int attention_v1_launch(hipStream_t st, const AttnParams& p, const AttnPlan& pl);
 int attention_v2_launch(hipStream_t st, const AttnParams& p, const AttnPlan& pl);
 int attention_long_launch(hipStream_t st, const AttnParams& p, const AttnPlan& pl);
+constexpr int attn_keep_rows(int n_t) { return 16 * n_t; }
+size_t attn_keep_bits_bytes(const AttnParams& p);
+int attention_keep_bits_launch(hipStream_t st, const AttnParams& p);
 inline int attn_unplanned(const char* what) { set_error("attention: %s is not instantiated and attn_plan never plans it", what); return MDT_ERR_UNSUPPORTED; }
 
 constexpr bool attn_head_dim_ok(int hd) { return hd == 16 || hd == 64 || hd == 96 || hd == 128; }
diff --git a/multimodaldiscussiontransformer_amd/csrc/attention_v2.hip b/multimodaldiscussiontransformer_amd/csrc/attention_v2.hip
--- a/multimodaldiscussiontransformer_amd/csrc/attention_v2.hip
+++ b/multimodaldiscussiontransformer_amd/csrc/attention_v2.hip
@@ -119,6 +119,25 @@
 }
 __device__ __forceinline__ void row_piece(bf16_t* p, const f32x4& x, float scale) {
   *(bf16x4*)p = bf16x4{(bf16_t)(x[0] * scale), (bf16_t)(x[1] * scale), (bf16_t)(x[2] * scale), (bf16_t)(x[3] * scale)};
+}
+
+template <int B>
+__device__ __forceinline__ uint32_t keep_mask(uint32_t w) {
+  uint32_t m;
+  asm("v_bfe_i32 %0, %1, %2, 1" : "=v"(m) : "v"(w), "n"(B));
+  return m;
+}
+__device__ __forceinline__ float keep_and(float x, uint32_t m) { return __builtin_bit_cast(float, __builtin_bit_cast(uint32_t, x) & m); }
+__device__ __forceinline__ void v2_p_ds_bits(f32x4& sc, f32x4& dp, float scale2, float kb, const f32x4& l2v, const f32x4& dlv, uint32_t nib) {
+  const uint32_t m[4] = {keep_mask<0>(nib), keep_mask<1>(nib), keep_mask<2>(nib), keep_mask<3>(nib)};
+#pragma unroll
+  for (int r = 0; r < 4; ++r) {
+    const float v = __builtin_fmaf(sc[r], scale2, kb);
+    const float p = __builtin_amdgcn_exp2f(v - l2v[r]);
+    const float dpv = keep_and(dp[r], m[r]);
+    sc[r] = keep_and(p, m[r]);
+    dp[r] = p * (dpv - dlv[r]);
+  }
 }
 
 template <bool STRUCT>
@@ -986,10 +1005,11 @@
   attn_bwd_v4_body<HD, DROP, true>(P, rows_img, ldq);
 }
 
-template <int HD, bool DROP, int NU>
+template <int HD, bool DROP, int NU, bool KB = false>
 __device__ __forceinline__ void v5_phase1(const AttnParams& P, const bf16_t* img0, const bf16_t* img1, const float* s_kb, const float* s_lse,
                                           const float* s_delta, bf16_t* dsT, int ldq, const bf16x8 (&wk)[2][v2_ks<HD>], const bf16x8 (&wv)[2][v2_ks<HD>],
-                                          int wave, int lane, int S, int SL, int drop_bh, int n_tq, bf16_t* dqkv, int64_t gld, int D, float ik) {
+                                          int wave, int lane, int S, int SL, int drop_bh, int n_tq, bf16_t* dqkv, int64_t gld, int D, float ik,
+                                          const uint64_t (&wkb)[2]) {
   constexpr int ND = HD / 16;
   const mdt_attn_fwd_args& a = P.f;
   const int g = lane >> 4, c = lane & 15, odd = c & 1;
@@ -1043,9 +1063,12 @@
 #pragma unroll
         for (int t = 0; t < 2; ++t) {
           const int qb = (t0 + t) * 16 + 4 * g;
-          bool keep[4] = {true, true, true, true};
-          if constexpr (DROP) attn_keep4_queries(P.drop, kh[u], qb, s2h, odd, keep);
-          v2_p_ds<false>(sc[u][t], dp[u][t], scale2, kb[u], l2v[t], dlv[t], keep);
+          if constexpr (KB) v2_p_ds_bits(sc[u][t], dp[u][t], scale2, kb[u], l2v[t], dlv[t], (uint32_t)(wkb[u] >> (4 * (t0 + t))));
+          else {
+            bool keep[4] = {true, true, true, true};
+            if constexpr (DROP) attn_keep4_queries(P.drop, kh[u], qb, s2h, odd, keep);
+            v2_p_ds<false>(sc[u][t], dp[u][t], scale2, kb[u], l2v[t], dlv[t], keep);
+          }
         }
         fp[u] = v2_pack(sc[u][0], sc[u][1]);
         fs[u] = v2_pack(dp[u][0], dp[u][1]);
@@ -1083,8 +1106,9 @@
   return v;
 }
 
-template <int HD, bool DROP>
-__global__ __launch_bounds__(512) __attribute__((amdgpu_waves_per_eu(2, 2))) void attn_bwd_v5_kernel(AttnParams P, int rows_img, int ldq, int n_items) {
+template <int HD, bool DROP, bool KB>
+__device__ __forceinline__ void attn_bwd_v5_body(const AttnParams& P, int rows_img, int ldq, int n_items) {
+  static_assert(!KB || DROP, "bits are dropout decisions");
   constexpr int NCH = 4;
   extern __shared__ __attribute__((aligned(16))) char smem[];
   const mdt_attn_fwd_args& a = P.f;
@@ -1099,10 +1123,11 @@
   bf16_t* dsT = (bf16_t*)(s_delta + rows_img);
   const float ik = DROP ? P.drop.inv_keep : 1.0f, rik = 1.0f / ik;
 
-  int seq, h, S, n_t, rows_live, q_rows;
+  int seq, h, S, n_t, rows_live, q_rows, item_ix;
   int64_t row0;
   auto item_of = [&](int it_) {
     const int it = __builtin_amdgcn_readfirstlane(it_);
+    item_ix = it;
     const int si = it / a.H;
     h = it - si * a.H;
     seq = a.seq_ids ? v5_sload(a.seq_ids + si) : si;
@@ -1116,13 +1141,14 @@
     }
     n_t = (S + 15) >> 4;
     rows_live = ((n_t + 1) >> 1) * 32;
-    if (rows_live > rows_img || S <= 0) { S = 0; n_t = 0; rows_live = 0; }
+    if (rows_live > rows_img || S <= 0 || (KB && S > P.keep_rows)) { S = 0; n_t = 0; rows_live = 0; }
     q_rows = (a.q_limit > 0 && ((a.q_limit + 15) & ~15) < S) ? ((a.q_limit + 15) & ~15) : S;
   };
   bf16x8 cq[NCH], cg[NCH], co[NCH];
   float lv = 0.f;
   KeyBytes kbv{1, 0};
   bf16x8 wk[2][v2_ks<HD>], wv[2][v2_ks<HD>];
+  uint64_t wkb[2] = {0, 0};
   auto request_rows = [&](int tid) {
     if (S > 0) {
       const bf16_t* qkv = (const bf16_t*)a.qkv + row0 * a.ld_qkv + h * HD;
@@ -1143,6 +1169,14 @@
           wk[u][ks] = v2_frag_glb<HD>(qkv + D, tld, S, (wave + 8 * u) * 16, ks * 32, lane);
           wv[u][ks] = v2_frag_glb<HD>(qkv + 2 * D, tld, S, (wave + 8 * u) * 16, ks * 32, lane);
         }
+      if constexpr (KB) {
+        const uint64_t* kbk = attn_keep_item(P, item_ix) + (lane >> 4);
+#pragma unroll
+        for (int u = 0; u < 2; ++u) {
+          const int kr = (wave + 8 * u) * 16 + (lane & 15);
+          wkb[u] = kbk[(kr < P.keep_rows ? kr : P.keep_rows - 1) * 4];
+        }
+      }
     }
   };
 
@@ -1160,6 +1194,7 @@
     for (int u = 0; u < 2; ++u)
 #pragma unroll
       for (int ks = 0; ks < v2_ks<HD>; ++ks) asm volatile("" ::"v"(wk[u][ks]), "v"(wv[u][ks]));
+    if constexpr (KB) asm volatile("" ::"v"(wkb[0]), "v"(wkb[1]));
     __syncthreads();
     const int nxt = it + (int)gridDim.x;
     const bool more = nxt < n_items;
@@ -1167,8 +1202,8 @@
     bf16_t* dqkv = (bf16_t*)P.dqkv + c_row0 * P.ld_dqkv + c_h * HD;
     const int n_tq = (a.q_limit > 0 && ((a.q_limit + 15) >> 4) < c_nt) ? (a.q_limit + 15) >> 4 : c_nt;
     const int lane1 = v5_opaque(lane);
-    if (wave + 8 < c_nt) v5_phase1<HD, DROP, 2>(P, img0, img1, s_kb, s_lse, s_delta, dsT, ldq, wk, wv, wave, lane1, cS, SL, c_seq * a.H + c_h, n_tq, dqkv, gld, D, ik);
-    else if (wave < c_nt) v5_phase1<HD, DROP, 1>(P, img0, img1, s_kb, s_lse, s_delta, dsT, ldq, wk, wv, wave, lane1, cS, SL, c_seq * a.H + c_h, n_tq, dqkv, gld, D, ik);
+    if (wave + 8 < c_nt) v5_phase1<HD, DROP, 2, KB>(P, img0, img1, s_kb, s_lse, s_delta, dsT, ldq, wk, wv, wave, lane1, cS, SL, c_seq * a.H + c_h, n_tq, dqkv, gld, D, ik, wkb);
+    else if (wave < c_nt) v5_phase1<HD, DROP, 1, KB>(P, img0, img1, s_kb, s_lse, s_delta, dsT, ldq, wk, wv, wave, lane1, cS, SL, c_seq * a.H + c_h, n_tq, dqkv, gld, D, ik, wkb);
     __syncthreads();
     const int tid2 = v5_opaque(tid), lane2 = tid2 & 63;
 #pragma unroll
@@ -1182,11 +1217,22 @@
     __syncthreads();
   }
 }
+template <int HD, bool DROP>
+__global__ __launch_bounds__(512) __attribute__((amdgpu_waves_per_eu(2, 2))) void attn_bwd_v5_kernel(AttnParams P, int rows_img, int ldq, int n_items) {
+  attn_bwd_v5_body<HD, DROP, false>(P, rows_img, ldq, n_items);
+}
+template <int HD>
+__global__ __launch_bounds__(512) __attribute__((amdgpu_waves_per_eu(2, 2))) void attn_bwd_v5kb_kernel(AttnParams P, int rows_img, int ldq, int n_items) {
+  attn_bwd_v5_body<HD, true, true>(P, rows_img, ldq, n_items);
+}
 
 template <bool DROP>
 static int launch_one_pass(hipStream_t st, const AttnParams& p, const AttnPlan& pl) {
   const dim3 grid(p.f.H, p.f.nseq);
   const size_t lds = attn_one_pass_lds_bytes(pl.n_t);
+  if constexpr (DROP) {
+    if (p.f.keep_bits) return launch_route<attn_bwd_v5kb_kernel<64>>("v5", dim3((unsigned)pl.wgs), 512, lds, st, p, pl.rows_img, pl.ldq, pl.items);
+  }
   if (pl.route == AttnRoute::v5) return launch_route<attn_bwd_v5_kernel<64, DROP>>("v5", dim3((unsigned)pl.wgs), 512, lds, st, p, pl.rows_img, pl.ldq, pl.items);
   if (pl.route == AttnRoute::v4x) return launch_route<attn_bwd_v4x_kernel<64, DROP>>("v4x", grid, pl.waves * 64, lds, st, p, pl.rows_img, pl.ldq);
   return launch_route<attn_bwd_v4_kernel<64, DROP>>("v4", grid, pl.waves * 64, lds, st, p, pl.rows_img, pl.ldq);
diff --git a/multimodaldiscussiontransformer_amd/engine.py b/multimodaldiscussiontransformer_amd/engine.py
--- a/multimodaldiscussiontransformer_amd/engine.py
+++ b/multimodaldiscussiontransformer_amd/engine.py
@@ -328,6 +328,7 @@
 
 
 _WGRAD_ASUM = os.environ.get("MDT_WGRAD_ASUM", "1") != "0"
+_ATTN_KEEP_BITS = os.environ.get("MDT_ATTN_KEEP_BITS", "1") != "0"
 
 
 def wgrad(tape: Tape, dy: torch.Tensor, x: torch.Tensor, w: torch.nn.Parameter, b: Optional[torch.nn.Parameter]):
@@ -502,6 +503,7 @@
                 lt_ = lora_fwd(P, src, qkv_)
                 if tape.inference:
                     lt_ = None
+            kb_ = ops.attention_keep_bits(qkv_, spec.nseq, spec.S, spec.H, **kw) if (_ATTN_KEEP_BITS and p_attn > 0 and not tape.inference) else None
             ctx_full_, lse_ = ops.attention_fwd(qkv_, spec.nseq, spec.S, spec.H, **kw)
             ctx_, xk = gather(ctx_full_), gather(xd)
             t_ = ops.gemm(ctx_, P.o_w.data, bias=P.o_b.data, residual=xk, drop_p=p_hidden, drop_seed=s_o)
@@ -510,7 +512,7 @@
                 ops.lora_up_add_drop(lto, Lo.Bt.data, t_, alpha=Lo.scale, drop_p=p_hidden, drop_seed=s_o)
                 if not tape.inference:
                     lts["o"] = lto
-            return qkv_, lt_, ctx_full_, lse_, ctx_, t_
+            return qkv_, lt_, ctx_full_, lse_, ctx_, t_, kb_
 
         def fc2_fwd(h_, h8, res):
             y_ = linear(f8, h_, P.fc2_w, "fc2", x8=h8, bias=P.fc2_b.data, residual=res, drop_p=p_hidden, drop_seed=s_f2)[0]
@@ -546,13 +548,13 @@
         lts = {}
         if not pre_ln:
             a_in = xd
-            qkv, lt, ctx_full, lse, ctx, t = attn_fwd(a_in, None)
+            qkv, lt, ctx_full, lse, ctx, t, kb = attn_fwd(a_in, None)
             f_in, m1, r1, f_in8 = ln8(t, P.ln1_w, P.ln1_b, P.fc1_w, "fc1")
             u, h, y = ffn_fwd(f_in, f_in8, f_in)
             out, m2, r2 = ops.layernorm_fwd(y, P.ln2_w.data, P.ln2_b.data, eps)
         else:
             a_in, m1, r1, a_in8 = ln8(xd, P.ln1_w, P.ln1_b, P.qkv_w, "qkv")
-            qkv, lt, ctx_full, lse, ctx, t = attn_fwd(a_in, a_in8)
+            qkv, lt, ctx_full, lse, ctx, t, kb = attn_fwd(a_in, a_in8)
             f_in, m2, r2, f_in8 = ln8(t, P.ln2_w, P.ln2_b, P.fc1_w, "fc1")
             u, h, out = ffn_fwd(f_in, f_in8, t)
         if policy == "ffn":
@@ -590,7 +592,7 @@
             dctx = ops.gemm(dtd, P.o_w.data, trans_b=True)
             if Lo is not None:
                 lora_dense_bwd(tape, Lo, ctx, lts["o"], dtd, dctx)
-            dqkv = _attention_bwd(tape, spec, kw, dctx, qkv, ctx_full, lse, spread)
+            dqkv = _attention_bwd(tape, spec, kw, dctx, qkv, ctx_full, lse, spread, keep_bits=kb)
             wgrad(tape, dqkv, a_in, P.qkv_w, P.qkv_b)
             dx_ = dgrad(dqkv, P.qkv_w, residual=None if dres is None else spread(dres)) if want_dx else None
             if P.lora_A is not None:
@@ -633,7 +635,7 @@
     return o
 
 
-def _attention_bwd(tape: Tape, spec: AttnSpec, kw: dict, dctx, qkv, ctx, lse, spread=lambda g: g):
+def _attention_bwd(tape: Tape, spec: AttnSpec, kw: dict, dctx, qkv, ctx, lse, spread=lambda g: g, keep_bits=None):
     extra = {}
     if spec.sp_table is not None and _DETERMINISTIC:
         return _attention_bwd_ordered(tape, spec, kw, dctx, qkv, ctx, lse, spread)
@@ -642,7 +644,7 @@
                      d_virt=None if tape.pgrad(spec.virt) is None else tape.pgrad(spec.virt).view(-1))
     want_dense = spec.dense_bias_var is not None and spec.dense_bias_var.needs_grad
     dqkv, dbias = ops.attention_bwd(spread(dctx), qkv, ctx, lse, spec.nseq, spec.S, spec.H, **kw, want_dense_dbias=want_dense,
-                                    **extra)
+                                    keep_bits=keep_bits, **extra)
     if want_dense:
         tape.add_grad(spec.dense_bias_var, dbias)
     return dqkv
diff --git a/multimodaldiscussiontransformer_amd/ops.py b/multimodaldiscussiontransformer_amd/ops.py
--- a/multimodaldiscussiontransformer_amd/ops.py
+++ b/multimodaldiscussiontransformer_amd/ops.py
@@ -12,7 +12,7 @@
 
 __all__ = [
     "bert_embed_rows",
-    "gemm", "colsum", "layernorm_fwd", "layernorm_bwd", "attention_fwd", "attention_bwd", "attention_mean_probs", "graph_attn_bias",
+    "gemm", "colsum", "layernorm_fwd", "layernorm_bwd", "attention_fwd", "attention_bwd", "attention_keep_bits", "attention_mean_probs", "graph_attn_bias",
     "row_axpby", "row_scatter_add", "bert_embed_sum", "bert_embed_ln_rows", "vit_patchify", "vit_assemble", "vit_patch_embed", "graph_node_feature",
     "tanh_fwd", "tanh_bwd", "node_ce", "contrastive_loss", "fp8_quantize", "fp8_scale_update", "gemm_fp8", "cast", "transpose2d", "dropout", "dropout_mask",
     "sum_slices", "gemm_splitk_ordered", "colsum_ordered", "layernorm_bwd_ordered", "segments_of", "row_segment_sum",
@@ -160,6 +160,35 @@
     return name.value.decode(), (geo[0], geo[1])
 
 
+def _attn_keep(a, keep_bits, i):
+    if keep_bits is not None and keep_bits[i] is not None:
+        assert keep_bits[i].dtype == torch.uint8 and keep_bits[i].is_contiguous()
+        a.keep_bits, a.keep_bits_bytes = ptr(keep_bits[i]), keep_bits[i].numel()
+
+
+def attention_keep_bits(qkv, nseq, S, H, *, seq_stride=None, pos_stride=1, scale=None, key_mask=None, dense_bias=None,
+                        attn_bias=None, spatial_pos=None, sp_table=None, virt=None, key_pad=None, drop_p=0.0, drop_seed=0,
+                        seq_offsets=None, q_limit=0, bins=None, always=False):
+    made, any_ = [], False
+    for ids, cap in _attn_bins(bins, qkv, H, S):
+        b = L.AttnBwdArgs()
+        b.f = _attn_args(qkv, qkv, qkv, nseq, S, H, None, seq_stride, pos_stride, scale, key_mask, dense_bias, attn_bias, spatial_pos,
+                         sp_table, virt, key_pad, drop_p, drop_seed, seq_offsets, q_limit, ids, cap)
+        b.dout, b.ld_dout = ptr(qkv), _2d(qkv)
+        b.dqkv, b.ld_dqkv = ptr(qkv), _2d(qkv)
+        n = int(lib.mdt_attention_keep_bits_bytes(C.byref(b)))
+        if always:
+            n = b.f.nseq * H * 16 * (((cap or S) + 15) // 16) * 32
+        if n == 0:
+            made.append(None)
+            continue
+        bits = torch.empty(n, dtype=torch.uint8, device=qkv.device)
+        check(lib.mdt_attention_keep_bits(stream(), C.byref(b), ptr(bits), n), "mdt_attention_keep_bits")
+        made.append(bits)
+        any_ = True
+    return made if any_ else None
+
+
 def attention_fwd(qkv, nseq, S, H, *, seq_stride=None, pos_stride=1, scale=None, key_mask=None, dense_bias=None,
                   attn_bias=None, spatial_pos=None, sp_table=None, virt=None, key_pad=None, drop_p=0.0, drop_seed=0,
                   seq_offsets=None, q_limit=0, bins=None, out=None, lse=None):
@@ -201,7 +230,7 @@
 def attention_bwd(dout, qkv, out, lse, nseq, S, H, *, seq_stride=None, pos_stride=1, scale=None, key_mask=None,
                   dense_bias=None, attn_bias=None, spatial_pos=None, sp_table=None, virt=None, key_pad=None,
                   want_dense_dbias=False, d_sp_table=None, d_virt=None, drop_p=0.0, drop_seed=0, seq_offsets=None, q_limit=0,
-                  bins=None, dqkv=None, dbias=None):
+                  bins=None, dqkv=None, dbias=None, keep_bits=None):
     D = qkv.shape[1] // 3
     if dqkv is None:
         dqkv = torch.empty(qkv.shape, dtype=qkv.dtype, device=qkv.device)
@@ -212,10 +241,11 @@
         dbias = _f32_out(dbias, (nseq, H, S, S), qkv.device).zero_()
     elif want_dense_dbias:
         dbias = torch.zeros(nseq, H, S, S, dtype=torch.float32, device=qkv.device)
-    for ids, cap in _attn_bins(bins, qkv, H, S):
+    for i, (ids, cap) in enumerate(_attn_bins(bins, qkv, H, S)):
         b = L.AttnBwdArgs()
         b.f = _attn_args(qkv, out, lse, nseq, S, H, None, seq_stride, pos_stride, scale, key_mask, dense_bias, attn_bias, spatial_pos,
                          sp_table, virt, key_pad, drop_p, drop_seed, seq_offsets, q_limit, ids, cap)
+        _attn_keep(b.f, keep_bits, i)
         b.dout, b.ld_dout = ptr(dout), _2d(dout)
         b.dqkv, b.ld_dqkv = ptr(dqkv), _2d(dqkv)
         b.d_dense_bias = ptr(dbias)
```
